# rail-berkeley/serl

Hardware: NVIDIA H100
Metric: drq_critic_grad_steps_per_sec (higher is better)
Workload: dtype f16

## Files before the change

serl_b200/csrc/conv3x3_res.cu:

```cuda
#include "common.cuh"
#include "conv_common.cuh"
#include "serl_b200.h"
#include "wgmma.cuh"

namespace serl {

template <int W, int CI>
struct R3Cfg {
  static constexpr int ROWS = 256 / W;
  static constexpr int BANDS = W / ROWS;
  static constexpr int PARTS = BANDS * (CI / 64);
  static constexpr int CB = CI / 64;
  static constexpr int NBOX = 3 * CB;
  static constexpr int STAGES = CB == 1 ? 3 : 2;
  static constexpr int BOX = W * (ROWS + 2) * 128;
  static constexpr int WTILES = 9 * CB;
  static constexpr int CG = CI / 4;
  static constexpr int NG = 64 / CG;
  static constexpr int WPG = CG / 16;
  static constexpr int PF = 4;
  static constexpr int OFF_A = WTILES * 8192;
  static constexpr int OFF_STG = OFF_A + STAGES * BOX;
  static constexpr int OFF_RED = OFF_STG + 8 * 1024;
  static constexpr int OFF_SLOT = OFF_RED + 2 * 4 * 2 * 4;
  static constexpr int OFF_BAR = OFF_SLOT + 4 * BANDS * NG * 2 * 4;
  static constexpr int SMEM = OFF_BAR + 8 * (2 * STAGES + 5) + 1024;
  static_assert(ROWS * W == 256 && (BOX % 1024) == 0 && SMEM <= 232448, "conv3x3_res_kernel: shared memory layout");
};

struct Res3Args {
  uint16_t* y; const uint16_t* res; const float* gamma; const float* beta;
  const float* res_stats; const float* res_gamma; const float* res_beta;
  int32_t* error; int N, relu; float eps;
};

template <class F, int W, int CI>
__global__ void __launch_bounds__(CONV_THREADS, 1)
conv3x3_res_kernel(const __grid_constant__ CUtensorMap xmap, const __grid_constant__ CUtensorMap wmap, const Res3Args a) {
  pdl_prologue();
  using K = R3Cfg<W, CI>;
  extern __shared__ uint8_t smem_raw[];
  uint8_t* smem = reinterpret_cast<uint8_t*>((reinterpret_cast<uintptr_t>(smem_raw) + 1023) & ~(uintptr_t)1023);
  uint8_t* sW = smem;
  uint8_t* sA = smem + K::OFF_A;
  float* red = reinterpret_cast<float*>(smem + K::OFF_RED);
  float* slot = reinterpret_cast<float*>(smem + K::OFF_SLOT);
  uint64_t* full = reinterpret_cast<uint64_t*>(smem + K::OFF_BAR);
  uint64_t* empty = full + K::STAGES;
  uint64_t* wbar = empty + K::STAGES;
  uint64_t* gnbar = wbar + 1;

  const int warp = threadIdx.x >> 5, lane = threadIdx.x & 31;
  const int part = blockIdx.x % K::PARTS;
  const int band = part % K::BANDS, n0 = (part / K::BANDS) * 64;
  const int row0 = band * K::ROWS;
  const int img0 = blockIdx.x / K::PARTS, img_step = gridDim.x / K::PARTS;

  if (threadIdx.x == 0) {
    for (int s = 0; s < K::STAGES; ++s) { tc_mbar_init(&full[s], 1); tc_mbar_init(&empty[s], 4); }
    tc_mbar_init(wbar, 1);
    for (int q = 0; q < 4; ++q) tc_mbar_init(&gnbar[q], 1);
    asm volatile("fence.mbarrier_init.release.cluster;" ::: "memory");
  }
  __syncthreads();
  if constexpr (K::BANDS > 1) cluster_sync_all();

  if (warp >= 8) {
    asm volatile("setmaxnreg.dec.sync.aligned.u32 40;" ::: "memory");
    if (warp == 8 && lane == 0) {
      asm volatile("prefetch.tensormap [%0];" ::"l"(&xmap) : "memory");
      asm volatile("prefetch.tensormap [%0];" ::"l"(&wmap) : "memory");
      tc_mbar_expect_tx(wbar, (uint32_t)(K::WTILES * 8192));
      for (int t = 0; t < K::WTILES; ++t) tc_tma_2d(sW + t * 8192, &wmap, t * 64, n0, wbar);
      bool ok = true;
      int it = 0;
      for (int n = img0; n < a.N && ok; n += img_step)
        for (int b = 0; b < K::NBOX; ++b, ++it) {
          const int s = it % K::STAGES;
          ok = tc_mbar_wait(&empty[s], ((uint32_t)(it / K::STAGES) & 1u) ^ 1u, a.error);
          if (!ok) break;
          tc_mbar_expect_tx(&full[s], (uint32_t)K::BOX);
          tc_tma_4d(sA + s * K::BOX, &xmap, (b / 3) * 64, b % 3 - 1, row0 - 1, n, &full[s]);
        }
    }
  } else {
    asm volatile("setmaxnreg.inc.sync.aligned.u32 232;" ::: "memory");
    const int g = warp >> 2, wl = warp & 3, tid = threadIdx.x & 127;
    const uint32_t a_base = smem_u32(sA), w_base = smem_u32(sW);
    const float count = (float)(W * W) * (float)K::CG;
    const int grp = wl / K::WPG;
    const int cl = 16 * wl + (lane >> 2);
    uint8_t* stg = smem + K::OFF_STG + warp * 1024;
    const uint32_t mrow = smem_u32(stg) + (uint32_t)(((lane >> 4) * 8 + (lane & 7)) * 32 + ((((lane >> 3) ^ (lane >> 2)) & 1) << 4));
    const int gpx = lane >> 1, gh = lane & 1;
    const uint32_t grow = (uint32_t)(gpx * 32 + ((gh ^ (gpx >> 2)) & 1) * 16);
    bool ok = tc_mbar_wait(wbar, 0u, a.error);
    ok = mma_bar_and(ok);
    float acc[128];
    for (int m = 0;; ++m) {
      const int i = g + 2 * m;
      const int n = img0 + i * img_step;
      if (n >= a.N) break;
      if (i > 0) named_bar_sync(2 + g, 256);
      int it = i * K::NBOX;
      for (int b = 0; b < K::NBOX && ok; ++b, ++it) {
        const int s = it % K::STAGES;
        ok = tc_mbar_wait(&full[s], (uint32_t)(it / K::STAGES) & 1u, a.error);
        if (!ok) break;
        const int cb = b / 3, sx = b % 3;
        const uint32_t bs = a_base + (uint32_t)(s * K::BOX);
        wg_fence();
#pragma unroll
        for (int r = 0; r < 3; ++r) {
          const uint32_t ws = w_base + (uint32_t)(((r * 3 + sx) * K::CB + cb) * 8192);
#pragma unroll
          for (int k = 0; k < 4; ++k)
            wg_mma_h16_n256<F::kBf16>(acc, wg_desc(ws) + 2 * k, wg_desc(bs + (uint32_t)(r * W * 128)) + 2 * k, (uint32_t)(b | r | k));
        }
        wg_commit();
        if (b > 0) {
          wg_wait<1>();
          __syncwarp();
          if (lane == 0) tc_mbar_arrive(&empty[(it - 1) % K::STAGES]);
        }
      }
      if (n + img_step < a.N) named_bar_arrive(3 - g, 256);

      const size_t pix0 = (size_t)n * W * W + (size_t)row0 * W;
      const uint16_t* rsrc = a.res + (pix0 + gpx) * CI + n0 + 16 * wl + 8 * gh;
      uint4 rbuf[K::PF][2];
      if (a.res && ok) {
#pragma unroll
        for (int p = 0; p < K::PF; ++p)
#pragma unroll
          for (int e = 0; e < 2; ++e) rbuf[p][e] = __ldg(reinterpret_cast<const uint4*>(rsrc + (size_t)(32 * p + 16 * e) * CI));
      }
      wg_wait<0>();
      __syncwarp();
      if (ok && lane == 0) tc_mbar_arrive(&empty[(it - 1) % K::STAGES]);

      float S = 0.f, SS = 0.f;
#pragma unroll
      for (int j = 0; j < 32; ++j) {
        const float* d = &acc[4 * j];
        S += (d[0] + d[1]) + (d[2] + d[3]);
        SS += (d[0] * d[0] + d[1] * d[1]) + (d[2] * d[2] + d[3] * d[3]);
      }
      S = warp_sum(S); SS = warp_sum(SS);
      if constexpr (K::WPG > 1) {
        if (lane == 0) *reinterpret_cast<float2*>(red + (g * 4 + wl) * 2) = make_float2(S, SS);
        named_bar_sync(4 + g, 128);
        S = 0.f; SS = 0.f;
#pragma unroll
        for (int k = 0; k < K::WPG; ++k) {
          const float2 v = *reinterpret_cast<const float2*>(red + (g * 4 + grp * K::WPG + k) * 2);
          S += v.x; SS += v.y;
        }
      }
      if constexpr (K::BANDS > 1) {
        const int q = 2 * g + (m & 1);
        if (ok) {
          if (tid == 0) tc_mbar_expect_tx(&gnbar[q], (uint32_t)(K::BANDS * K::NG * 2 * 4));
          if (lane < 2) {
            const float v = lane ? SS : S;
            float* dst = slot + ((q * K::BANDS + band) * K::NG + grp) * 2 + lane;
#pragma unroll
            for (int rk = 0; rk < K::BANDS; ++rk) {
              uint32_t rdst, rbar;
              asm volatile("mapa.shared::cluster.u32 %0, %1, %2;" : "=r"(rdst) : "r"(smem_u32(dst)), "r"(rk));
              asm volatile("mapa.shared::cluster.u32 %0, %1, %2;" : "=r"(rbar) : "r"(smem_u32(&gnbar[q])), "r"(rk));
              asm volatile("st.async.shared::cluster.mbarrier::complete_tx::bytes.b32 [%0], %1, [%2];"
                           ::"r"(rdst), "r"(__float_as_uint(v)), "r"(rbar) : "memory");
            }
          }
          ok = tc_mbar_wait_cluster(&gnbar[q], (uint32_t)(m >> 1) & 1u, a.error);
        }
        S = 0.f; SS = 0.f;
#pragma unroll
        for (int rk = 0; rk < K::BANDS; ++rk) {
          S += slot[((q * K::BANDS + rk) * K::NG + grp) * 2];
          SS += slot[((q * K::BANDS + rk) * K::NG + grp) * 2 + 1];
        }
      }
      if (!ok) continue;

      const float mean = S / count;
      const float var = fmaxf(SS / count - mean * mean, 0.f);
      const float rstd = rsqrtf(var + a.eps);
      float ga[2], gb[2], ra[2] = {1.f, 1.f}, rb[2] = {0.f, 0.f};
#pragma unroll
      for (int h = 0; h < 2; ++h) {
        const int c = n0 + cl + 8 * h;
        ga[h] = rstd * a.gamma[c];
        gb[h] = a.beta[c] - mean * ga[h];
      }
      if (a.res_stats) {
        const int rg = (n0 + cl) / K::CG;
        const float rs = a.res_stats[((size_t)n * 4 + rg) * 2], rss = a.res_stats[((size_t)n * 4 + rg) * 2 + 1];
        const float rmean = rs / count;
        const float rvar = fmaxf(rss / count - rmean * rmean, 0.f);
        const float rrstd = rsqrtf(rvar + a.eps);
#pragma unroll
        for (int h = 0; h < 2; ++h) {
          const int c = n0 + cl + 8 * h;
          ra[h] = rrstd * a.res_gamma[c];
          rb[h] = a.res_beta[c] - rmean * ra[h];
        }
      }

      uint16_t* ydst = a.y + (pix0 + gpx) * CI + n0 + 16 * wl + 8 * gh;
#pragma unroll
      for (int rd = 0; rd < 8; ++rd) {
        uint32_t rv[2][4];
        if (a.res) {
#pragma unroll
          for (int e = 0; e < 2; ++e) *reinterpret_cast<uint4*>(stg + grow + e * 512) = rbuf[rd % K::PF][e];
          __syncwarp();
          ldsm_x4_trans(mrow, rv[0]);
          ldsm_x4_trans(mrow + 512, rv[1]);
          if (rd + K::PF < 8) {
#pragma unroll
            for (int e = 0; e < 2; ++e)
              rbuf[rd % K::PF][e] = __ldg(reinterpret_cast<const uint4*>(rsrc + (size_t)(32 * (rd + K::PF) + 16 * e) * CI));
          }
        }
        uint32_t o[2][4];
#pragma unroll
        for (int x = 0; x < 2; ++x)
#pragma unroll
          for (int jj = 0; jj < 2; ++jj)
#pragma unroll
            for (int h = 0; h < 2; ++h) {
              const float* d = &acc[4 * (4 * rd + 2 * x + jj) + 2 * h];
              float o0 = fmaf(d[0], ga[h], gb[h]), o1 = fmaf(d[1], ga[h], gb[h]);
              if (a.res) {
                const float2 r = F::unpack(rv[x][2 * jj + h]);
                o0 += a.res_stats ? fmaf(r.x, ra[h], rb[h]) : r.x;
                o1 += a.res_stats ? fmaf(r.y, ra[h], rb[h]) : r.y;
              }
              if (a.relu) { o0 = fmaxf(o0, 0.f); o1 = fmaxf(o1, 0.f); }
              o[x][2 * jj + h] = F::pack(o0, o1);
            }
        __syncwarp();
        stsm_x4_trans(mrow, o[0]);
        stsm_x4_trans(mrow + 512, o[1]);
        __syncwarp();
#pragma unroll
        for (int e = 0; e < 2; ++e)
          *reinterpret_cast<uint4*>(ydst + (size_t)(32 * rd + 16 * e) * CI) = *reinterpret_cast<const uint4*>(stg + grow + e * 512);
        __syncwarp();
      }
    }
  }
  if constexpr (K::BANDS > 1) cluster_sync_all();
}

template <class F, int W, int CI>
static int launch_conv3x3_res(const serl_conv3x3_res_desc* d, cudaStream_t st) {
  using K = R3Cfg<W, CI>;
  auto kern = conv3x3_res_kernel<F, W, CI>;
  static int groups = 0;
  if (!groups) {
    if (cudaFuncSetAttribute(kern, cudaFuncAttributeMaxDynamicSharedMemorySize, K::SMEM) != cudaSuccess) return check_launch("cudaFuncSetAttribute(conv3x3_res)");
    int dev = 0, sms = 0, n = 0;
    cudaGetDevice(&dev);
    cudaDeviceGetAttribute(&sms, cudaDevAttrMultiProcessorCount, dev);
    if (K::BANDS > 1) {
      cudaLaunchConfig_t cfg = {};
      cudaLaunchAttribute attr[1];
      attr[0].id = cudaLaunchAttributeClusterDimension;
      attr[0].val.clusterDim.x = K::BANDS; attr[0].val.clusterDim.y = 1; attr[0].val.clusterDim.z = 1;
      cfg.gridDim = dim3(K::BANDS * sms); cfg.blockDim = dim3(CONV_THREADS); cfg.dynamicSmemBytes = K::SMEM;
      cfg.attrs = attr; cfg.numAttrs = 1;
      if (cudaOccupancyMaxActiveClusters(&n, kern, &cfg) != cudaSuccess) return check_launch("cudaOccupancyMaxActiveClusters(conv3x3_res)");
    } else {
      int per_sm = 0;
      if (cudaOccupancyMaxActiveBlocksPerMultiprocessor(&per_sm, kern, CONV_THREADS, K::SMEM) != cudaSuccess) return check_launch("cudaOccupancyMaxActiveBlocksPerMultiprocessor(conv3x3_res)");
      n = per_sm * sms / K::PARTS;
    }
    if (n <= 0) { set_last_error("serl_conv3x3_res_h16: conv3x3_res_kernel (%d B shared memory) cannot be resident", K::SMEM); return SERL_ERR_CUDA; }
    groups = n;
  }
  TcEncodeTiledFn enc = tc_get_encode();
  if (!enc) { set_last_error("serl_conv3x3_res_h16: cuTensorMapEncodeTiled unavailable"); return SERL_ERR_CUDA; }
  const CUtensorMapDataType dt = d->fmt == SERL_FMT_FP16 ? CU_TENSOR_MAP_DATA_TYPE_FLOAT16 : CU_TENSOR_MAP_DATA_TYPE_BFLOAT16;
  CUtensorMap xmap, wmap;
  {
    const cuuint64_t gdim[4] = {(cuuint64_t)CI, (cuuint64_t)W, (cuuint64_t)W, (cuuint64_t)d->N};
    const cuuint64_t gstr[3] = {(cuuint64_t)CI * 2, (cuuint64_t)W * CI * 2, (cuuint64_t)W * W * CI * 2};
    const cuuint32_t box[4] = {64u, (cuuint32_t)W, (cuuint32_t)(K::ROWS + 2), 1u};
    const cuuint32_t estr[4] = {1u, 1u, 1u, 1u};
    CUresult r = enc(&xmap, dt, 4, const_cast<void*>(d->x), gdim, gstr, box, estr, CU_TENSOR_MAP_INTERLEAVE_NONE, CU_TENSOR_MAP_SWIZZLE_128B,
                     CU_TENSOR_MAP_L2_PROMOTION_L2_256B, CU_TENSOR_MAP_FLOAT_OOB_FILL_NONE);
    if (r != CUDA_SUCCESS) { set_last_error("serl_conv3x3_res_h16: cuTensorMapEncodeTiled (input) failed (%d)", (int)r); return SERL_ERR_CUDA; }
  }
  {
    const cuuint64_t gdim[2] = {(cuuint64_t)9 * CI, (cuuint64_t)CI};
    const cuuint64_t gstr[1] = {(cuuint64_t)9 * CI * 2};
    const cuuint32_t box[2] = {64u, 64u};
    const cuuint32_t estr[2] = {1u, 1u};
    CUresult r = enc(&wmap, dt, 2, const_cast<void*>(d->w), gdim, gstr, box, estr, CU_TENSOR_MAP_INTERLEAVE_NONE, CU_TENSOR_MAP_SWIZZLE_128B,
                     CU_TENSOR_MAP_L2_PROMOTION_L2_256B, CU_TENSOR_MAP_FLOAT_OOB_FILL_NONE);
    if (r != CUDA_SUCCESS) { set_last_error("serl_conv3x3_res_h16: cuTensorMapEncodeTiled (weights) failed (%d)", (int)r); return SERL_ERR_CUDA; }
  }
  Res3Args a{};
  a.y = static_cast<uint16_t*>(d->y); a.res = static_cast<const uint16_t*>(d->res); a.gamma = d->gamma; a.beta = d->beta;
  a.res_stats = d->res_stats; a.res_gamma = d->res_gamma; a.res_beta = d->res_beta;
  a.error = d->error; a.N = d->N; a.relu = d->relu; a.eps = d->eps;
  const int rounds = ceil_div(d->N, groups);
  const int used = ceil_div(d->N, rounds);
  launch_k_cluster(kern, dim3(used * K::PARTS), dim3(CONV_THREADS), K::BANDS, (size_t)K::SMEM, st, xmap, wmap, a);
  return check_launch("conv3x3_res_kernel");
}

template <int S, int WO, int CI>
struct PPCfg {
  static constexpr int CO = S * CI;
  static constexpr int HW = WO * WO;
  static constexpr int IMGS = 256 / HW;
  static constexpr int NSL = CO / 64;
  static constexpr int CB = CI / 64;
  static constexpr int NB = S == 2 ? 6 : 3;
  static constexpr int NPH = S == 2 ? 2 : 1;
  static constexpr int BROWS = WO + (S == 2 ? 1 : 2);
  static constexpr int SHIFT = IMGS * WO * 128;
  static constexpr int BOX = BROWS * SHIFT;
  static constexpr int STAGE = BOX + (S == 2 ? 2 : 3) * 8192;
  static constexpr int STAGES = S == 2 ? 4 : 3;
  static constexpr int CG = CO / 4;
  static constexpr int WPG = CG / 16;
  static constexpr int PF = 4;
  static constexpr int OFF_STG = STAGES * STAGE;
  static constexpr int OFF_RED = OFF_STG + 8 * 1024;
  static constexpr int OFF_BAR = OFF_RED + 2 * 2 * 4 * IMGS * 2 * 4;
  static constexpr int SMEM = OFF_BAR + 8 * 2 * STAGES + 1024;
  static_assert(IMGS * HW == 256 && WPG <= 4 && (SHIFT % 1024) == 0 && (STAGE % 1024) == 0 && SMEM <= 232448,
                "conv3x3_pp_kernel: shared memory layout");
  static __host__ __device__ constexpr int nbox(int ph) { return ph ? CB : NB * CB; }
};

struct PPArgs {
  uint16_t* y; uint16_t* r; float* out_f32; const uint16_t* res;
  const float* gamma; const float* beta; const float* gamma_p; const float* beta_p;
  const float* res_stats; const float* res_gamma; const float* res_beta;
  int32_t* error; int N, relu; float eps;
};

template <class F, int S, int WO, int CI>
__global__ void __launch_bounds__(CONV_THREADS, 1)
conv3x3_pp_kernel(const __grid_constant__ CUtensorMap xmap, const __grid_constant__ CUtensorMap wmap,
                  const __grid_constant__ CUtensorMap pmap, const PPArgs a) {
  pdl_prologue();
  using K = PPCfg<S, WO, CI>;
  extern __shared__ uint8_t smem_raw[];
  uint8_t* smem = reinterpret_cast<uint8_t*>((reinterpret_cast<uintptr_t>(smem_raw) + 1023) & ~(uintptr_t)1023);
  float* red = reinterpret_cast<float*>(smem + K::OFF_RED);
  uint64_t* full = reinterpret_cast<uint64_t*>(smem + K::OFF_BAR);
  uint64_t* empty = full + K::STAGES;

  const int warp = threadIdx.x >> 5, lane = threadIdx.x & 31;
  const int n_items = ceil_div(a.N, K::IMGS) * K::NSL;
  auto item_of = [&](int P) {
    const int q = blockIdx.x + ((P & 1) + 2 * ((P >> 1) / K::NPH)) * gridDim.x;
    return P >= 0 && q < n_items ? q : -1;
  };
  auto past_end = [&](int P) { return blockIdx.x + 2 * ((P >> 1) / K::NPH) * gridDim.x >= n_items; };

  if (threadIdx.x == 0) {
    for (int s = 0; s < K::STAGES; ++s) { tc_mbar_init(&full[s], 1); tc_mbar_init(&empty[s], 4); }
    asm volatile("fence.mbarrier_init.release.cluster;" ::: "memory");
  }
  __syncthreads();

  if (warp >= 8) {
    asm volatile("setmaxnreg.dec.sync.aligned.u32 40;" ::: "memory");
    if (warp == 8 && lane == 0) {
      asm volatile("prefetch.tensormap [%0];" ::"l"(&xmap) : "memory");
      asm volatile("prefetch.tensormap [%0];" ::"l"(&wmap) : "memory");
      if (S == 2) asm volatile("prefetch.tensormap [%0];" ::"l"(&pmap) : "memory");
      bool ok = true;
      int it = 0;
      for (int P = 0; ok && !past_end(P); ++P) {
        const int q = item_of(P);
        if (q < 0) continue;
        const int ph = (P >> 1) % K::NPH;
        const int img0 = (q / K::NSL) * K::IMGS, n0 = (q % K::NSL) * 64;
        for (int b = 0; b < K::nbox(ph); ++b, ++it) {
          const int s = it % K::STAGES;
          ok = tc_mbar_wait(&empty[s], ((uint32_t)(it / K::STAGES) & 1u) ^ 1u, a.error);
          if (!ok) break;
          const int cb = ph ? b : b / K::NB, sx = ph ? 0 : b % 3, row0 = S == 2 && !ph ? (b % K::NB) / 3 : 0;
          const int ntap = ph ? 1 : S == 1 ? 3 : row0 == 0 ? 2 : 1;
          uint8_t* st = smem + s * K::STAGE;
          tc_mbar_expect_tx(&full[s], (uint32_t)(K::BOX + ntap * 8192));
          tc_tma_4d(st, &xmap, cb * 64, S == 2 ? sx : sx - 1, img0, S == 2 ? row0 : -1, &full[s]);
          for (int t = 0; t < ntap; ++t) {
            if (ph) tc_tma_2d(st + K::BOX, &pmap, cb * 64, n0, &full[s]);
            else tc_tma_2d(st + K::BOX + t * 8192, &wmap, (((S == 2 ? row0 + 2 * t : t) * 3 + sx) * K::CB + cb) * 64, n0, &full[s]);
          }
        }
      }
    }
  } else {
    asm volatile("setmaxnreg.inc.sync.aligned.u32 232;" ::: "memory");
    const int g = warp >> 2, wl = warp & 3;
    const uint32_t s_base = smem_u32(smem);
    const float count = (float)K::HW * (float)K::CG;
    const int grp = wl / K::WPG;
    const int cl = 16 * wl + (lane >> 2);
    uint8_t* stg = smem + K::OFF_STG + warp * 1024;
    const uint32_t mrow = smem_u32(stg) + (uint32_t)(((lane >> 4) * 8 + (lane & 7)) * 32 + ((((lane >> 3) ^ (lane >> 2)) & 1) << 4));
    const int gpx = lane >> 1, gh = lane & 1;
    const uint32_t grow = (uint32_t)(gpx * 32 + ((gh ^ (gpx >> 2)) & 1) * 16);
    const int pbase = K::IMGS == 1 ? gpx : gpx & 7;
    constexpr int RSTEP = K::IMGS == 1 ? 32 : 8, ESTEP = K::IMGS == 1 ? 16 : 0;
    auto im_of = [&](int e) { return K::IMGS == 1 ? 0 : 2 * e + (gpx >> 3); };
    bool ok = true;
    int it = 0;
    float acc[128];
    for (int P = 0; !past_end(P); ++P) {
      const int q = item_of(P);
      if (q < 0) continue;
      const int k = P >> 1, ph = k % K::NPH;
      if ((P & 1) != g) { it += K::nbox(ph); continue; }
      const int img0 = (q / K::NSL) * K::IMGS, n0 = (q % K::NSL) * 64;
      if (item_of(P - 1) >= 0) named_bar_sync(2 + g, 256);
      if (ph == 0) {
        for (int cb = 0; cb < K::CB && ok; ++cb) {
#pragma unroll
          for (int bb = 0; bb < K::NB; ++bb, ++it) {
            const int s = it % K::STAGES;
            ok = tc_mbar_wait(&full[s], (uint32_t)(it / K::STAGES) & 1u, a.error);
            if (!ok) break;
            const int ntap = S == 1 ? 3 : bb < 3 ? 2 : 1;
            const uint32_t bs = s_base + (uint32_t)(s * K::STAGE), ws = bs + (uint32_t)K::BOX;
            wg_fence();
#pragma unroll
            for (int t = 0; t < ntap; ++t)
#pragma unroll
              for (int kk = 0; kk < 4; ++kk)
                wg_mma_h16_n256<F::kBf16>(acc, wg_desc(ws + (uint32_t)(t * 8192)) + 2 * kk, wg_desc(bs + (uint32_t)(t * K::SHIFT)) + 2 * kk,
                                          (uint32_t)(cb | bb | t | kk));
            wg_commit();
            if (cb > 0 || bb > 0) {
              wg_wait<1>();
              __syncwarp();
              if (lane == 0) tc_mbar_arrive(&empty[(it - 1) % K::STAGES]);
            }
          }
        }
      } else {
        for (int cb = 0; cb < K::CB && ok; ++cb, ++it) {
          const int s = it % K::STAGES;
          ok = tc_mbar_wait(&full[s], (uint32_t)(it / K::STAGES) & 1u, a.error);
          if (!ok) break;
          const uint32_t bs = s_base + (uint32_t)(s * K::STAGE), ws = bs + (uint32_t)K::BOX;
          wg_fence();
#pragma unroll
          for (int kk = 0; kk < 4; ++kk)
            wg_mma_h16_n256<F::kBf16>(acc, wg_desc(ws) + 2 * kk, wg_desc(bs) + 2 * kk, (uint32_t)(cb | kk));
          wg_commit();
          if (cb > 0) {
            wg_wait<1>();
            __syncwarp();
            if (lane == 0) tc_mbar_arrive(&empty[(it - 1) % K::STAGES]);
          }
        }
      }
      if (item_of(P + 1) >= 0) named_bar_arrive(3 - g, 256);

      const uint16_t* rsrc = a.res + ((size_t)img0 * K::HW + pbase) * CI + n0 + 16 * wl + 8 * gh;
      uint4 rbuf[K::PF][2];
      if (S == 1 && a.res && ok) {
#pragma unroll
        for (int p = 0; p < K::PF; ++p)
#pragma unroll
          for (int e = 0; e < 2; ++e)
            rbuf[p][e] = img0 + im_of(e) < a.N ? __ldg(reinterpret_cast<const uint4*>(rsrc + (size_t)(im_of(e) * K::HW + p * RSTEP + e * ESTEP) * CI))
                                               : make_uint4(0u, 0u, 0u, 0u);
      }
      wg_wait<0>();
      __syncwarp();
      if (ok && lane == 0) tc_mbar_arrive(&empty[(it - 1) % K::STAGES]);

      float sm[K::IMGS], ss[K::IMGS];
#pragma unroll
      for (int im = 0; im < K::IMGS; ++im) { sm[im] = 0.f; ss[im] = 0.f; }
#pragma unroll
      for (int j = 0; j < 32; ++j) {
        const float* d = &acc[4 * j];
        sm[j % K::IMGS] += (d[0] + d[1]) + (d[2] + d[3]);
        ss[j % K::IMGS] += (d[0] * d[0] + d[1] * d[1]) + (d[2] * d[2] + d[3] * d[3]);
      }
      float* rw = red + (((k & 1) * 2 + g) * 4) * K::IMGS * 2;
#pragma unroll
      for (int im = 0; im < K::IMGS; ++im) {
        sm[im] = warp_sum(sm[im]); ss[im] = warp_sum(ss[im]);
        if (lane == 0) *reinterpret_cast<float2*>(rw + (wl * K::IMGS + im) * 2) = make_float2(sm[im], ss[im]);
      }
      named_bar_sync(4 + g, 128);
      if (!ok) continue;
      float mean[K::IMGS], rstd[K::IMGS];
#pragma unroll
      for (int im = 0; im < K::IMGS; ++im) {
        float s0 = 0.f, s1 = 0.f;
#pragma unroll
        for (int w = 0; w < K::WPG; ++w) {
          const float2 v = *reinterpret_cast<const float2*>(rw + ((grp * K::WPG + w) * K::IMGS + im) * 2);
          s0 += v.x; s1 += v.y;
        }
        mean[im] = s0 / count;
        rstd[im] = rsqrtf(fmaxf(s1 / count - mean[im] * mean[im], 0.f) + a.eps);
      }

      const float* gam = ph ? a.gamma_p : a.gamma;
      const float* bet = ph ? a.beta_p : a.beta;
      const bool relu = S == 2 ? ph == 0 : a.relu != 0;
      const bool rnorm = S == 1 && a.res_stats;
      float ga[K::IMGS][2], gb[K::IMGS][2], ra[K::IMGS][2], rb[K::IMGS][2];
#pragma unroll
      for (int im = 0; im < K::IMGS; ++im) {
        float rmean = 0.f, rrstd = 1.f;
        if (rnorm && img0 + im < a.N) {
          const float* rs = a.res_stats + ((size_t)(img0 + im) * 4 + n0 / K::CG) * 2;
          rmean = rs[0] / count;
          rrstd = rsqrtf(fmaxf(rs[1] / count - rmean * rmean, 0.f) + a.eps);
        }
#pragma unroll
        for (int h = 0; h < 2; ++h) {
          const int c = n0 + cl + 8 * h;
          ga[im][h] = rstd[im] * gam[c];
          gb[im][h] = bet[c] - mean[im] * ga[im][h];
          ra[im][h] = rnorm ? rrstd * a.res_gamma[c] : 1.f;
          rb[im][h] = rnorm ? a.res_beta[c] - rmean * ra[im][h] : 0.f;
        }
      }

      uint16_t* out = S == 2 && ph ? a.r : a.y;
      const size_t obase = ((size_t)img0 * K::HW + pbase) * K::CO + n0 + 16 * wl + 8 * gh;
#pragma unroll
      for (int rd = 0; rd < 8; ++rd) {
        uint32_t rv[2][4];
        if (S == 1 && a.res) {
#pragma unroll
          for (int e = 0; e < 2; ++e) *reinterpret_cast<uint4*>(stg + grow + e * 512) = rbuf[rd % K::PF][e];
          __syncwarp();
          ldsm_x4_trans(mrow, rv[0]);
          ldsm_x4_trans(mrow + 512, rv[1]);
          if (rd + K::PF < 8) {
#pragma unroll
            for (int e = 0; e < 2; ++e)
              if (img0 + im_of(e) < a.N)
                rbuf[rd % K::PF][e] = __ldg(reinterpret_cast<const uint4*>(rsrc + (size_t)(im_of(e) * K::HW + (rd + K::PF) * RSTEP + e * ESTEP) * CI));
          }
        }
        uint32_t o[2][4];
#pragma unroll
        for (int x = 0; x < 2; ++x)
#pragma unroll
          for (int jj = 0; jj < 2; ++jj) {
            const int j = 4 * rd + 2 * x + jj, im = j % K::IMGS;
#pragma unroll
            for (int h = 0; h < 2; ++h) {
              const float* d = &acc[4 * j + 2 * h];
              float o0 = fmaf(d[0], ga[im][h], gb[im][h]), o1 = fmaf(d[1], ga[im][h], gb[im][h]);
              if (S == 1 && a.res) {
                const float2 r = F::unpack(rv[x][2 * jj + h]);
                o0 += fmaf(r.x, ra[im][h], rb[im][h]);
                o1 += fmaf(r.y, ra[im][h], rb[im][h]);
              }
              if (relu) { o0 = fmaxf(o0, 0.f); o1 = fmaxf(o1, 0.f); }
              if (S == 1 && a.out_f32 && img0 + im < a.N) {
                float* of = a.out_f32 + ((size_t)(img0 + im) * K::HW + 8 * (j / K::IMGS) + 2 * (lane & 3)) * CI + n0 + cl + 8 * h;
                of[0] = o0;
                of[CI] = o1;
              }
              o[x][2 * jj + h] = F::pack(o0, o1);
            }
          }
        __syncwarp();
        if (S == 2 || !a.out_f32) {
          stsm_x4_trans(mrow, o[0]);
          stsm_x4_trans(mrow + 512, o[1]);
          __syncwarp();
#pragma unroll
          for (int e = 0; e < 2; ++e)
            if (img0 + im_of(e) < a.N)
              *reinterpret_cast<uint4*>(out + obase + (size_t)(im_of(e) * K::HW + rd * RSTEP + e * ESTEP) * K::CO) =
                  *reinterpret_cast<const uint4*>(stg + grow + e * 512);
          __syncwarp();
        }
      }
    }
  }
}

template <class F, int S, int WO, int CI>
static int launch_conv3x3_pp(const char* name, const void* x, const void* w, const void* w_proj, int fmt, const PPArgs& a, cudaStream_t st) {
  using K = PPCfg<S, WO, CI>;
  auto kern = conv3x3_pp_kernel<F, S, WO, CI>;
  static int slots = 0;
  if (!slots) {
    if (cudaFuncSetAttribute(kern, cudaFuncAttributeMaxDynamicSharedMemorySize, K::SMEM) != cudaSuccess) return check_launch("cudaFuncSetAttribute(conv3x3_pp)");
    int dev = 0, sms = 0, per_sm = 0;
    cudaGetDevice(&dev);
    cudaDeviceGetAttribute(&sms, cudaDevAttrMultiProcessorCount, dev);
    if (cudaOccupancyMaxActiveBlocksPerMultiprocessor(&per_sm, kern, CONV_THREADS, K::SMEM) != cudaSuccess) return check_launch("cudaOccupancyMaxActiveBlocksPerMultiprocessor(conv3x3_pp)");
    if (per_sm <= 0) { set_last_error("%s: conv3x3_pp_kernel (%d B shared memory) cannot be resident", name, K::SMEM); return SERL_ERR_CUDA; }
    slots = per_sm * sms;
  }
  TcEncodeTiledFn enc = tc_get_encode();
  if (!enc) { set_last_error("%s: cuTensorMapEncodeTiled unavailable", name); return SERL_ERR_CUDA; }
  const CUtensorMapDataType dt = fmt == SERL_FMT_FP16 ? CU_TENSOR_MAP_DATA_TYPE_FLOAT16 : CU_TENSOR_MAP_DATA_TYPE_BFLOAT16;
  CUtensorMap xmap, wmap, pmap;
  {
    constexpr int WI = S * WO;
    const cuuint64_t gdim[4] = {(cuuint64_t)CI, (cuuint64_t)WI, (cuuint64_t)a.N, (cuuint64_t)WI};
    const cuuint64_t gstr[3] = {(cuuint64_t)CI * 2, (cuuint64_t)WI * WI * CI * 2, (cuuint64_t)WI * CI * 2};
    const cuuint32_t box[4] = {64u, (cuuint32_t)(S * WO), (cuuint32_t)K::IMGS, (cuuint32_t)(S * K::BROWS)};
    const cuuint32_t estr[4] = {1u, (cuuint32_t)S, 1u, (cuuint32_t)S};
    CUresult r = enc(&xmap, dt, 4, const_cast<void*>(x), gdim, gstr, box, estr, CU_TENSOR_MAP_INTERLEAVE_NONE, CU_TENSOR_MAP_SWIZZLE_128B,
                     CU_TENSOR_MAP_L2_PROMOTION_L2_256B, CU_TENSOR_MAP_FLOAT_OOB_FILL_NONE);
    if (r != CUDA_SUCCESS) { set_last_error("%s: cuTensorMapEncodeTiled (input) failed (%d)", name, (int)r); return SERL_ERR_CUDA; }
  }
  for (int pj = 0; pj < S; ++pj) {
    const cuuint64_t kdim = (cuuint64_t)(pj ? 1 : 9) * CI;
    const cuuint64_t gdim[2] = {kdim, (cuuint64_t)K::CO};
    const cuuint64_t gstr[1] = {kdim * 2};
    const cuuint32_t box[2] = {64u, 64u};
    const cuuint32_t estr[2] = {1u, 1u};
    CUresult r = enc(pj ? &pmap : &wmap, dt, 2, const_cast<void*>(pj ? w_proj : w), gdim, gstr, box, estr, CU_TENSOR_MAP_INTERLEAVE_NONE,
                     CU_TENSOR_MAP_SWIZZLE_128B, CU_TENSOR_MAP_L2_PROMOTION_L2_256B, CU_TENSOR_MAP_FLOAT_OOB_FILL_NONE);
    if (r != CUDA_SUCCESS) { set_last_error("%s: cuTensorMapEncodeTiled (weights) failed (%d)", name, (int)r); return SERL_ERR_CUDA; }
  }
  if (S == 1) pmap = wmap;
  const int items = ceil_div(a.N, K::IMGS) * K::NSL;
  const int rounds = ceil_div(items, slots);
  launch_k(kern, dim3(ceil_div(items, rounds)), dim3(CONV_THREADS), (size_t)K::SMEM, st, xmap, wmap, pmap, a);
  return check_launch("conv3x3_pp_kernel");
}

template <class F, int WO, int CI>
static int launch_conv3x3s2_pp(const serl_conv3x3s2_res_desc* d, cudaStream_t st) {
  PPArgs a{};
  a.y = static_cast<uint16_t*>(d->y); a.r = static_cast<uint16_t*>(d->r);
  a.gamma = d->gamma; a.beta = d->beta; a.gamma_p = d->gamma_proj; a.beta_p = d->beta_proj;
  a.error = d->error; a.N = d->N; a.relu = 1; a.eps = d->eps;
  return launch_conv3x3_pp<F, 2, WO, CI>("serl_conv3x3s2_res_h16", d->x, d->w, d->w_proj, d->fmt, a, st);
}

template <class F>
static int launch_conv3x3_res8_pp(const serl_conv3x3_res_desc* d, cudaStream_t st) {
  PPArgs a{};
  a.out_f32 = d->out_f32; a.y = d->out_f32 ? nullptr : static_cast<uint16_t*>(d->y);
  a.res = static_cast<const uint16_t*>(d->res); a.gamma = d->gamma; a.beta = d->beta;
  a.res_stats = d->res_stats; a.res_gamma = d->res_gamma; a.res_beta = d->res_beta;
  a.error = d->error; a.N = d->N; a.relu = d->relu; a.eps = d->eps;
  return launch_conv3x3_pp<F, 1, 8, 256>("serl_conv3x3_res_h16", d->x, d->w, nullptr, d->fmt, a, st);
}

template <int WO, int CI>
struct S2Cfg {
  static constexpr int CO = 2 * CI;
  static constexpr int BN = 128;
  static constexpr int M = 128;
  static constexpr int HW = WO * WO;
  static constexpr int IMGS = M / HW;
  static constexpr int NSL = CO / BN;
  static constexpr int CB = CI / 64;
  static constexpr int NB = 9;
  static constexpr int NBOX = NB * CB;
  static constexpr int BOX = IMGS * HW * 128;
  static constexpr int TILE = BN * 128;
  static constexpr int STAGE = BOX + 2 * TILE;
  static constexpr int STAGES = 4;
  static constexpr int CG = CO / 4;
  static constexpr int CGS = 64;
  static constexpr int GPS = 64 / CGS;
  static constexpr int NGC = BN / CG;
  static constexpr int OFF_STG = STAGES * STAGE;
  static constexpr int OFF_PAR = OFF_STG + 8 * 1024;
  static constexpr int OFF_RED = OFF_PAR + BN * 16;
  static constexpr int OFF_ST = OFF_RED + 8 * 2 * GPS * 16;
  static constexpr int OFF_BAR = OFF_ST + IMGS * NGC * 16;
  static constexpr int SMEM = OFF_BAR + 8 * 2 * STAGES + 1024;
  static_assert(WO == 4 && BN % CG == 0, "conv3x3s2_res_kernel: the WO 4 head, an item holds whole GroupNorm groups");
  static_assert(M % HW == 0 && (BOX % 1024) == 0 && (STAGE % 1024) == 0 && SMEM <= 232448, "conv3x3s2_res_kernel: shared memory layout");
  __device__ static constexpr int m_off(int wg, int) { return wg * 64; }
  __device__ static constexpr int n_off(int h) { return h * 64; }
};

struct S2Args {
  uint16_t* y; uint16_t* r; const float* gamma; const float* beta; const float* gamma_p; const float* beta_p;
  int32_t* error; int N; float eps;
};

template <class F, int WO, int CI>
__global__ void __launch_bounds__(CONV_THREADS, 1)
conv3x3s2_res_kernel(const __grid_constant__ CUtensorMap xmap, const __grid_constant__ CUtensorMap wmap,
                     const __grid_constant__ CUtensorMap pmap, const S2Args a) {
  pdl_prologue();
  using K = S2Cfg<WO, CI>;
  extern __shared__ uint8_t smem_raw[];
  uint8_t* smem = reinterpret_cast<uint8_t*>((reinterpret_cast<uintptr_t>(smem_raw) + 1023) & ~(uintptr_t)1023);
  float* par = reinterpret_cast<float*>(smem + K::OFF_PAR);
  float* red = reinterpret_cast<float*>(smem + K::OFF_RED);
  float* gst = reinterpret_cast<float*>(smem + K::OFF_ST);
  uint64_t* full = reinterpret_cast<uint64_t*>(smem + K::OFF_BAR);
  uint64_t* empty = full + K::STAGES;

  const int warp = threadIdx.x >> 5, lane = threadIdx.x & 31;
  const int n_items = ceil_div(a.N, K::IMGS) * K::NSL;

  if (threadIdx.x == 0) {
    for (int s = 0; s < K::STAGES; ++s) { tc_mbar_init(&full[s], 1); tc_mbar_init(&empty[s], 8); }
    asm volatile("fence.mbarrier_init.release.cluster;" ::: "memory");
  }
  __syncthreads();

  if (warp >= 8) {
    asm volatile("setmaxnreg.dec.sync.aligned.u32 40;" ::: "memory");
    if (warp == 8 && lane == 0) {
      asm volatile("prefetch.tensormap [%0];" ::"l"(&xmap) : "memory");
      asm volatile("prefetch.tensormap [%0];" ::"l"(&wmap) : "memory");
      asm volatile("prefetch.tensormap [%0];" ::"l"(&pmap) : "memory");
      bool ok = true;
      int it = 0;
      for (int item = blockIdx.x; item < n_items && ok; item += gridDim.x) {
        const int img = (item / K::NSL) * K::IMGS, n0 = (item % K::NSL) * K::BN;
        for (int b = 0; b < K::NBOX; ++b, ++it) {
          const int s = it % K::STAGES;
          ok = tc_mbar_wait(&empty[s], ((uint32_t)(it / K::STAGES) & 1u) ^ 1u, a.error);
          if (!ok) break;
          const int cb = b / K::NB, row = (b % K::NB) / 3, sx = b % 3;
          const bool proj = row == 0 && sx == 0;
          uint8_t* st = smem + s * K::STAGE;
          tc_mbar_expect_tx(&full[s], (uint32_t)(K::BOX + (1 + (int)proj) * K::TILE));
          tc_tma_4d(st, &xmap, cb * 64, sx, row, img, &full[s]);
          tc_tma_2d(st + K::BOX, &wmap, ((row * 3 + sx) * K::CB + cb) * 64, n0, &full[s]);
          if (proj) tc_tma_2d(st + K::BOX + K::TILE, &pmap, cb * 64, n0, &full[s]);
        }
      }
    }
  } else {
    asm volatile("setmaxnreg.inc.sync.aligned.u32 232;" ::: "memory");
    const int tid = threadIdx.x, wg = tid >> 7, wl = warp & 3;
    const uint32_t s_base = smem_u32(smem);
    uint32_t a_off[2], b_off[2];
#pragma unroll
    for (int h = 0; h < 2; ++h) {
      const int m = K::m_off(wg, h);
      a_off[h] = (uint32_t)(m * 128);
      b_off[h] = (uint32_t)(K::n_off(h) * 128);
    }
    const float count = (float)K::HW * (float)K::CG;
    bool ok = true;
    int it = 0;
    float acc[2][32], pacc[2][32];
    for (int item = blockIdx.x; item < n_items && ok; item += gridDim.x) {
      const int img0 = (item / K::NSL) * K::IMGS, n0 = (item % K::NSL) * K::BN;
      for (int cb = 0; cb < K::CB && ok; ++cb) {
#pragma unroll
        for (int bb = 0; bb < K::NB; ++bb, ++it) {
          const int s = it % K::STAGES;
          ok = tc_mbar_wait(&full[s], (uint32_t)(it / K::STAGES) & 1u, a.error);
          if (!ok) break;
          const uint32_t as = s_base + (uint32_t)(s * K::STAGE), ws = as + (uint32_t)K::BOX;
          wg_fence();
#pragma unroll
          for (int k = 0; k < 4; ++k)
#pragma unroll
            for (int h = 0; h < 2; ++h)
              wg_mma_h16<F::kBf16>(acc[h], wg_desc(as + a_off[h]) + 2 * k, wg_desc(ws + b_off[h]) + 2 * k, (uint32_t)(cb | bb | k));
          if (bb == 0) {
#pragma unroll
            for (int k = 0; k < 4; ++k)
#pragma unroll
              for (int h = 0; h < 2; ++h)
                wg_mma_h16<F::kBf16>(pacc[h], wg_desc(as + a_off[h]) + 2 * k, wg_desc(ws + (uint32_t)K::TILE + b_off[h]) + 2 * k,
                                     (uint32_t)(cb | k));
          }
          wg_commit();
          if (cb > 0 || bb > 0) {
            wg_wait<1>();
            __syncwarp();
            if (lane == 0) tc_mbar_arrive(&empty[(it - 1) % K::STAGES]);
          }
        }
      }
      wg_wait<0>();
      ok = mma_bar_and(ok);
      if (!ok) break;
      __syncwarp();
      if (lane == 0) tc_mbar_arrive(&empty[(it - 1) % K::STAGES]);

#pragma unroll
      for (int h = 0; h < 2; ++h)
#pragma unroll
        for (int g = 0; g < K::GPS; ++g) {
          float v[4] = {0.f, 0.f, 0.f, 0.f};
#pragma unroll
          for (int j = g * K::CGS / 8; j < (g + 1) * K::CGS / 8; ++j) {
            const float* d = &acc[h][4 * j];
            const float* p = &pacc[h][4 * j];
            v[0] += (d[0] + d[1]) + (d[2] + d[3]);
            v[1] += (d[0] * d[0] + d[1] * d[1]) + (d[2] * d[2] + d[3] * d[3]);
            v[2] += (p[0] + p[1]) + (p[2] + p[3]);
            v[3] += (p[0] * p[0] + p[1] * p[1]) + (p[2] * p[2] + p[3] * p[3]);
          }
#pragma unroll
          for (int q = 0; q < 4; ++q) {
            v[q] = warp_sum(v[q]);
            if (lane == 0) red[((warp * 2 + h) * K::GPS + g) * 4 + q] = v[q];
          }
        }
      asm volatile("bar.sync 1, 256;" ::: "memory");
      if (tid < K::BN)
        *reinterpret_cast<float4*>(par + tid * 4) = make_float4(a.gamma[n0 + tid], a.beta[n0 + tid], a.gamma_p[n0 + tid], a.beta_p[n0 + tid]);
      if (tid < K::IMGS * K::NGC) {
        const int im = tid / K::NGC, gc = tid % K::NGC;
        float S[4] = {0.f, 0.f, 0.f, 0.f};
        for (int w = 0; w < 8; ++w)
          for (int h = 0; h < 2; ++h)
            for (int g = 0; g < K::GPS; ++g) {
              if ((K::m_off(w >> 2, h) + 16 * (w & 3)) / K::HW != im || (K::n_off(h) + g * K::CGS) / K::CG != gc) continue;
              for (int q = 0; q < 4; ++q) S[q] += red[((w * 2 + h) * K::GPS + g) * 4 + q];
            }
        const float mean = S[0] / count, pmean = S[2] / count;
        const float var = fmaxf(S[1] / count - mean * mean, 0.f), pvar = fmaxf(S[3] / count - pmean * pmean, 0.f);
        *reinterpret_cast<float4*>(gst + tid * 4) = make_float4(mean, rsqrtf(var + a.eps), pmean, rsqrtf(pvar + a.eps));
      }
      asm volatile("bar.sync 1, 256;" ::: "memory");

      uint8_t* stg = smem + K::OFF_STG + warp * 1024;
#pragma unroll
      for (int h = 0; h < 2; ++h)
#pragma unroll
        for (int hf = 0; hf < 2; ++hf) {
          const int m8 = K::m_off(wg, h) + wl * 16 + hf * 8;
          const int im = m8 / K::HW;
          if (img0 + im >= a.N) continue;
          const int rr = lane >> 2;
          const size_t pix0 = (size_t)img0 * K::HW + m8;
#pragma unroll 1
          for (int o = 0; o < 2; ++o) {
#pragma unroll
            for (int j = 0; j < 8; ++j) {
              const int c = K::n_off(h) + 8 * j + 2 * (lane & 3);
              const float4 sv = *reinterpret_cast<const float4*>(gst + (im * K::NGC + c / K::CG) * 4);
              const float4 p0 = *reinterpret_cast<const float4*>(par + c * 4), p1 = *reinterpret_cast<const float4*>(par + c * 4 + 4);
              float o0, o1;
              if (o == 0) {
                const float g0 = sv.y * p0.x, g1 = sv.y * p1.x;
                o0 = fmaxf(fmaf(acc[h][4 * j + 2 * hf], g0, p0.y - sv.x * g0), 0.f);
                o1 = fmaxf(fmaf(acc[h][4 * j + 2 * hf + 1], g1, p1.y - sv.x * g1), 0.f);
              } else {
                const float g0 = sv.w * p0.z, g1 = sv.w * p1.z;
                o0 = fmaf(pacc[h][4 * j + 2 * hf], g0, p0.w - sv.z * g0);
                o1 = fmaf(pacc[h][4 * j + 2 * hf + 1], g1, p1.w - sv.z * g1);
              }
              *reinterpret_cast<uint32_t*>(stg + rr * 128 + ((j ^ rr) << 4) + (lane & 3) * 4) = F::pack(o0, o1);
            }
            __syncwarp();
            uint16_t* out = o == 0 ? a.y : a.r;
#pragma unroll
            for (int e = lane; e < 64; e += 32) {
              const int q = e >> 3, ch = e & 7;
              const uint4 v = *reinterpret_cast<const uint4*>(stg + q * 128 + ((ch ^ q) << 4));
              *reinterpret_cast<uint4*>(out + (pix0 + q) * K::CO + n0 + K::n_off(h) + ch * 8) = v;
            }
            __syncwarp();
          }
        }
    }
  }
}

template <class F, int WO, int CI>
static int launch_conv3x3s2_res(const serl_conv3x3s2_res_desc* d, cudaStream_t st) {
  using K = S2Cfg<WO, CI>;
  auto kern = conv3x3s2_res_kernel<F, WO, CI>;
  static int slots = 0;
  if (!slots) {
    if (cudaFuncSetAttribute(kern, cudaFuncAttributeMaxDynamicSharedMemorySize, K::SMEM) != cudaSuccess) return check_launch("cudaFuncSetAttribute(conv3x3s2_res)");
    int dev = 0, sms = 0, per_sm = 0;
    cudaGetDevice(&dev);
    cudaDeviceGetAttribute(&sms, cudaDevAttrMultiProcessorCount, dev);
    if (cudaOccupancyMaxActiveBlocksPerMultiprocessor(&per_sm, kern, CONV_THREADS, K::SMEM) != cudaSuccess) return check_launch("cudaOccupancyMaxActiveBlocksPerMultiprocessor(conv3x3s2_res)");
    if (per_sm <= 0) { set_last_error("serl_conv3x3s2_res_h16: conv3x3s2_res_kernel (%d B shared memory) cannot be resident", K::SMEM); return SERL_ERR_CUDA; }
    slots = per_sm * sms;
  }
  TcEncodeTiledFn enc = tc_get_encode();
  if (!enc) { set_last_error("serl_conv3x3s2_res_h16: cuTensorMapEncodeTiled unavailable"); return SERL_ERR_CUDA; }
  const CUtensorMapDataType dt = d->fmt == SERL_FMT_FP16 ? CU_TENSOR_MAP_DATA_TYPE_FLOAT16 : CU_TENSOR_MAP_DATA_TYPE_BFLOAT16;
  CUtensorMap xmap, wmap, pmap;
  {
    const cuuint64_t gdim[4] = {(cuuint64_t)CI, (cuuint64_t)(2 * WO), (cuuint64_t)(2 * WO), (cuuint64_t)d->N};
    const cuuint64_t gstr[3] = {(cuuint64_t)CI * 2, (cuuint64_t)2 * WO * CI * 2, (cuuint64_t)4 * WO * WO * CI * 2};
    const cuuint32_t box[4] = {64u, (cuuint32_t)(2 * WO), (cuuint32_t)(2 * WO), (cuuint32_t)K::IMGS};
    const cuuint32_t estr[4] = {1u, 2u, 2u, 1u};
    CUresult r = enc(&xmap, dt, 4, const_cast<void*>(d->x), gdim, gstr, box, estr, CU_TENSOR_MAP_INTERLEAVE_NONE, CU_TENSOR_MAP_SWIZZLE_128B,
                     CU_TENSOR_MAP_L2_PROMOTION_L2_256B, CU_TENSOR_MAP_FLOAT_OOB_FILL_NONE);
    if (r != CUDA_SUCCESS) { set_last_error("serl_conv3x3s2_res_h16: cuTensorMapEncodeTiled (input) failed (%d)", (int)r); return SERL_ERR_CUDA; }
  }
  for (int pj = 0; pj < 2; ++pj) {
    const cuuint64_t kdim = (cuuint64_t)(pj ? 1 : 9) * CI;
    const cuuint64_t gdim[2] = {kdim, (cuuint64_t)K::CO};
    const cuuint64_t gstr[1] = {kdim * 2};
    const cuuint32_t box[2] = {64u, (cuuint32_t)K::BN};
    const cuuint32_t estr[2] = {1u, 1u};
    CUresult r = enc(pj ? &pmap : &wmap, dt, 2, const_cast<void*>(pj ? d->w_proj : d->w), gdim, gstr, box, estr, CU_TENSOR_MAP_INTERLEAVE_NONE,
                     CU_TENSOR_MAP_SWIZZLE_128B, CU_TENSOR_MAP_L2_PROMOTION_L2_256B, CU_TENSOR_MAP_FLOAT_OOB_FILL_NONE);
    if (r != CUDA_SUCCESS) { set_last_error("serl_conv3x3s2_res_h16: cuTensorMapEncodeTiled (weights) failed (%d)", (int)r); return SERL_ERR_CUDA; }
  }
  S2Args a{};
  a.y = static_cast<uint16_t*>(d->y); a.r = static_cast<uint16_t*>(d->r);
  a.gamma = d->gamma; a.beta = d->beta; a.gamma_p = d->gamma_proj; a.beta_p = d->beta_proj;
  a.error = d->error; a.N = d->N; a.eps = d->eps;
  const int items = ceil_div(d->N, K::IMGS) * K::NSL;
  const int rounds = ceil_div(items, slots);
  launch_k(kern, dim3(ceil_div(items, rounds)), dim3(CONV_THREADS), (size_t)K::SMEM, st, xmap, wmap, pmap, a);
  return check_launch("conv3x3s2_res_kernel");
}

template <int W, int CI>
struct DeepCfg {
  static constexpr int BN = 128;
  static constexpr int HW = W * W;
  static constexpr int IMGS = 256 / HW;
  static constexpr int NSL = CI / BN;
  static constexpr int CB = CI / 64;
  static constexpr int NB = 9;
  static constexpr int NBOX = NB * CB;
  static constexpr int BOX = IMGS * HW * 128;
  static constexpr int TILE = BN * 128;
  static constexpr int STAGE = BOX + TILE;
  static constexpr int STAGES = 4;
  static constexpr int RES = 128 * 128 * 2;
  static constexpr int RPS = STAGE / RES;
  static constexpr int NRES = 2 / RPS;
  static constexpr int CG = CI / 4;
  static constexpr int NGC = BN / CG;
  static constexpr int OFF_STG = STAGES * STAGE;
  static constexpr int OFF_PAR = OFF_STG + 8 * 2048;
  static constexpr int OFF_RED = OFF_PAR + BN * 16;
  static constexpr int OFF_ST = OFF_RED + 8 * 2 * 2 * 8;
  static constexpr int OFF_BAR = OFF_ST + IMGS * NGC * 16;
  static constexpr int SMEM = OFF_BAR + 8 * 2 * STAGES + 1024;
  static_assert(CG >= 64 && BN % CG == 0, "conv3x3_deep_kernel: an n64 sub-tile lies in one group, an item holds whole groups");
  static_assert(RPS >= 1 && NRES < STAGES, "conv3x3_deep_kernel: the residual fits the ring");
  static_assert(HW >= 16 && (BOX % 1024) == 0 && (STAGE % 1024) == 0 && SMEM <= 232448, "conv3x3_deep_kernel: shared memory layout");
  __device__ static constexpr int m_off(int wg, int h) { return wg * 128 + h * 64; }
};

struct DeepArgs {
  uint16_t* y; float* out_f32; const uint16_t* res; const float* gamma; const float* beta;
  const float* res_stats; const float* res_gamma; const float* res_beta;
  int32_t* error; int N, relu; float eps;
};

template <class F, int W, int CI>
__global__ void __launch_bounds__(CONV_THREADS, 1)
conv3x3_deep_kernel(const __grid_constant__ CUtensorMap xmap, const __grid_constant__ CUtensorMap wmap,
                    const __grid_constant__ CUtensorMap rmap, const DeepArgs a) {
  pdl_prologue();
  using K = DeepCfg<W, CI>;
  extern __shared__ uint8_t smem_raw[];
  uint8_t* smem = reinterpret_cast<uint8_t*>((reinterpret_cast<uintptr_t>(smem_raw) + 1023) & ~(uintptr_t)1023);
  float* par = reinterpret_cast<float*>(smem + K::OFF_PAR);
  float* red = reinterpret_cast<float*>(smem + K::OFF_RED);
  float* gst = reinterpret_cast<float*>(smem + K::OFF_ST);
  uint64_t* full = reinterpret_cast<uint64_t*>(smem + K::OFF_BAR);
  uint64_t* empty = full + K::STAGES;

  const int warp = threadIdx.x >> 5, lane = threadIdx.x & 31;
  const int n_items = ceil_div(a.N, K::IMGS) * K::NSL;

  if (threadIdx.x == 0) {
    for (int s = 0; s < K::STAGES; ++s) { tc_mbar_init(&full[s], 1); tc_mbar_init(&empty[s], 8); }
    asm volatile("fence.mbarrier_init.release.cluster;" ::: "memory");
  }
  __syncthreads();

  if (warp >= 8) {
    asm volatile("setmaxnreg.dec.sync.aligned.u32 40;" ::: "memory");
    if (warp == 8 && lane == 0) {
      asm volatile("prefetch.tensormap [%0];" ::"l"(&xmap) : "memory");
      asm volatile("prefetch.tensormap [%0];" ::"l"(&wmap) : "memory");
      if (a.res) asm volatile("prefetch.tensormap [%0];" ::"l"(&rmap) : "memory");
      bool ok = true;
      int it = 0;
      for (int item = blockIdx.x; item < n_items && ok; item += gridDim.x) {
        const int img = (item / K::NSL) * K::IMGS, n0 = (item % K::NSL) * K::BN;
        for (int b = 0; b < K::NBOX + (a.res ? K::NRES : 0); ++b, ++it) {
          const int s = it % K::STAGES;
          ok = tc_mbar_wait(&empty[s], ((uint32_t)(it / K::STAGES) & 1u) ^ 1u, a.error);
          if (!ok) break;
          uint8_t* st = smem + s * K::STAGE;
          if (b >= K::NBOX) {
            tc_mbar_expect_tx(&full[s], (uint32_t)(K::RPS * K::RES));
            for (int q = 0; q < K::RPS; ++q)
              for (int c = 0; c < 2; ++c)
                tc_tma_2d(st + q * K::RES + c * (K::RES / 2), &rmap, n0 + c * 64, img * K::HW + ((b - K::NBOX) * K::RPS + q) * 128, &full[s]);
            continue;
          }
          const int cb = b / K::NB, row = (b % K::NB) / 3, sx = b % 3;
          tc_mbar_expect_tx(&full[s], (uint32_t)K::STAGE);
          tc_tma_4d(st, &xmap, cb * 64, sx - 1, row - 1, img, &full[s]);
          tc_tma_2d(st + K::BOX, &wmap, ((row * 3 + sx) * K::CB + cb) * 64, n0, &full[s]);
        }
      }
    }
  } else {
    asm volatile("setmaxnreg.inc.sync.aligned.u32 232;" ::: "memory");
    const int tid = threadIdx.x, wg = tid >> 7, wl = warp & 3;
    const uint32_t s_base = smem_u32(smem);
    uint32_t a_off[2];
#pragma unroll
    for (int h = 0; h < 2; ++h) a_off[h] = (uint32_t)(K::m_off(wg, h) * 128);
    const float count = (float)K::HW * (float)K::CG;
    bool ok = true;
    int it = 0;
    float acc[2][2][32];
    for (int item = blockIdx.x; item < n_items && ok; item += gridDim.x) {
      const int img0 = (item / K::NSL) * K::IMGS, n0 = (item % K::NSL) * K::BN;
      for (int cb = 0; cb < K::CB && ok; ++cb) {
#pragma unroll
        for (int bb = 0; bb < K::NB; ++bb, ++it) {
          const int s = it % K::STAGES;
          ok = tc_mbar_wait(&full[s], (uint32_t)(it / K::STAGES) & 1u, a.error);
          if (!ok) break;
          const uint32_t as = s_base + (uint32_t)(s * K::STAGE), ws = as + (uint32_t)K::BOX;
          wg_fence();
#pragma unroll
          for (int k = 0; k < 4; ++k)
#pragma unroll
            for (int h = 0; h < 2; ++h)
#pragma unroll
              for (int c = 0; c < 2; ++c)
                wg_mma_h16<F::kBf16>(acc[h][c], wg_desc(as + a_off[h]) + 2 * k, wg_desc(ws + (uint32_t)(c * 64 * 128)) + 2 * k,
                                     (uint32_t)(cb | bb | k));
          wg_commit();
          if (cb > 0 || bb > 0) {
            wg_wait<1>();
            __syncwarp();
            if (lane == 0) tc_mbar_arrive(&empty[(it - 1) % K::STAGES]);
          }
        }
      }
      wg_wait<0>();
      ok = mma_bar_and(ok);
      if (!ok) break;
      __syncwarp();
      if (lane == 0) tc_mbar_arrive(&empty[(it - 1) % K::STAGES]);

#pragma unroll
      for (int h = 0; h < 2; ++h)
#pragma unroll
        for (int c = 0; c < 2; ++c) {
          float v0 = 0.f, v1 = 0.f;
#pragma unroll
          for (int j = 0; j < 8; ++j) {
            const float* d = &acc[h][c][4 * j];
            v0 += (d[0] + d[1]) + (d[2] + d[3]);
            v1 += (d[0] * d[0] + d[1] * d[1]) + (d[2] * d[2] + d[3] * d[3]);
          }
          v0 = warp_sum(v0); v1 = warp_sum(v1);
          if (lane == 0) *reinterpret_cast<float2*>(red + ((warp * 2 + h) * 2 + c) * 2) = make_float2(v0, v1);
        }
      asm volatile("bar.sync 1, 256;" ::: "memory");
      if (tid < K::BN) {
        const int ch = n0 + tid;
        *reinterpret_cast<float4*>(par + tid * 4) = a.res_stats ? make_float4(a.gamma[ch], a.beta[ch], a.res_gamma[ch], a.res_beta[ch])
                                                                : make_float4(a.gamma[ch], a.beta[ch], 1.f, 0.f);
      }
      if (tid < K::IMGS * K::NGC) {
        const int im = tid / K::NGC, gc = tid % K::NGC;
        float S = 0.f, SS = 0.f;
        for (int w = 0; w < 8; ++w)
          for (int h = 0; h < 2; ++h)
            for (int c = 0; c < 2; ++c) {
              if ((K::m_off(w >> 2, h) + 16 * (w & 3)) / K::HW != im || c * 64 / K::CG != gc) continue;
              S += red[((w * 2 + h) * 2 + c) * 2];
              SS += red[((w * 2 + h) * 2 + c) * 2 + 1];
            }
        const float mean = S / count;
        const float var = fmaxf(SS / count - mean * mean, 0.f);
        float rmean = 0.f, rrstd = 1.f;
        if (a.res_stats && img0 + im < a.N) {
          const float* rs = a.res_stats + ((size_t)(img0 + im) * 4 + (n0 / K::CG + gc)) * 2;
          rmean = rs[0] / count;
          rrstd = rsqrtf(fmaxf(rs[1] / count - rmean * rmean, 0.f) + a.eps);
        }
        *reinterpret_cast<float4*>(gst + tid * 4) = make_float4(mean, rsqrtf(var + a.eps), rmean, rrstd);
      }
      const int rpos = it + wg / K::RPS;
      const uint8_t* rsm = smem + (rpos % K::STAGES) * K::STAGE + (wg % K::RPS) * K::RES;
      if (a.res) ok = tc_mbar_wait(&full[rpos % K::STAGES], (uint32_t)(rpos / K::STAGES) & 1u, a.error);
      ok = mma_bar_and(ok);
      if (!ok) break;

      uint8_t* stg = smem + K::OFF_STG + warp * 2048;
      const int rr = lane >> 2;
#pragma unroll
      for (int h = 0; h < 2; ++h)
#pragma unroll
        for (int hf = 0; hf < 2; ++hf) {
          const int m8 = K::m_off(wg, h) + wl * 16 + hf * 8;
          const int im = m8 / K::HW;
          if (img0 + im >= a.N) continue;
          const size_t pix0 = (size_t)img0 * K::HW + m8;
#pragma unroll
          for (int c = 0; c < 2; ++c) {
            const float4 sv = *reinterpret_cast<const float4*>(gst + (im * K::NGC + c * 64 / K::CG) * 4);
#pragma unroll
            for (int j = 0; j < 8; ++j) {
              const int cl = c * 64 + 8 * j + 2 * (lane & 3);
              const float4 p0 = *reinterpret_cast<const float4*>(par + cl * 4), p1 = *reinterpret_cast<const float4*>(par + cl * 4 + 4);
              const float g0 = sv.y * p0.x, g1 = sv.y * p1.x;
              float o0 = fmaf(acc[h][c][4 * j + 2 * hf], g0, p0.y - sv.x * g0);
              float o1 = fmaf(acc[h][c][4 * j + 2 * hf + 1], g1, p1.y - sv.x * g1);
              if (a.res) {
                const float2 rv = F::unpack(*reinterpret_cast<const uint32_t*>(
                    rsm + c * (K::RES / 2) + (m8 - wg * 128 + rr) * 128 + ((j ^ rr) << 4) + (lane & 3) * 4));
                if (a.res_stats) {
                  const float r0 = sv.w * p0.z, r1 = sv.w * p1.z;
                  o0 += fmaf(rv.x, r0, p0.w - sv.z * r0);
                  o1 += fmaf(rv.y, r1, p1.w - sv.z * r1);
                } else {
                  o0 += rv.x; o1 += rv.y;
                }
              }
              if (a.relu) { o0 = fmaxf(o0, 0.f); o1 = fmaxf(o1, 0.f); }
              if (a.out_f32)
                *reinterpret_cast<float2*>(stg + rr * 256 + ((j ^ rr) << 5) + (lane & 3) * 8) = make_float2(o0, o1);
              else
                *reinterpret_cast<uint32_t*>(stg + rr * 128 + ((j ^ rr) << 4) + (lane & 3) * 4) = F::pack(o0, o1);
            }
            __syncwarp();
            if (a.out_f32) {
#pragma unroll
              for (int e = lane; e < 128; e += 32) {
                const int q = e >> 4, ch = e & 15;
                const uint4 v = *reinterpret_cast<const uint4*>(stg + q * 256 + (((ch >> 1) ^ q) << 5) + (ch & 1) * 16);
                *reinterpret_cast<uint4*>(a.out_f32 + (pix0 + q) * CI + n0 + c * 64 + ch * 4) = v;
              }
            } else {
#pragma unroll
              for (int e = lane; e < 64; e += 32) {
                const int q = e >> 3, ch = e & 7;
                const uint4 v = *reinterpret_cast<const uint4*>(stg + q * 128 + ((ch ^ q) << 4));
                *reinterpret_cast<uint4*>(a.y + (pix0 + q) * CI + n0 + c * 64 + ch * 8) = v;
              }
            }
            __syncwarp();
          }
        }
      if (a.res) {
        __syncwarp();
        if (lane == 0)
          for (int p = 0; p < K::NRES; ++p) tc_mbar_arrive(&empty[(it + p) % K::STAGES]);
        it += K::NRES;
      }
    }
  }
}

template <class F, int W, int CI>
static int launch_conv3x3_deep(const serl_conv3x3_res_desc* d, cudaStream_t st) {
  using K = DeepCfg<W, CI>;
  auto kern = conv3x3_deep_kernel<F, W, CI>;
  static int slots = 0;
  if (!slots) {
    if (cudaFuncSetAttribute(kern, cudaFuncAttributeMaxDynamicSharedMemorySize, K::SMEM) != cudaSuccess) return check_launch("cudaFuncSetAttribute(conv3x3_deep)");
    int dev = 0, sms = 0, per_sm = 0;
    cudaGetDevice(&dev);
    cudaDeviceGetAttribute(&sms, cudaDevAttrMultiProcessorCount, dev);
    if (cudaOccupancyMaxActiveBlocksPerMultiprocessor(&per_sm, kern, CONV_THREADS, K::SMEM) != cudaSuccess) return check_launch("cudaOccupancyMaxActiveBlocksPerMultiprocessor(conv3x3_deep)");
    if (per_sm <= 0) { set_last_error("serl_conv3x3_res_h16: conv3x3_deep_kernel (%d B shared memory) cannot be resident", K::SMEM); return SERL_ERR_CUDA; }
    slots = per_sm * sms;
  }
  TcEncodeTiledFn enc = tc_get_encode();
  if (!enc) { set_last_error("serl_conv3x3_res_h16: cuTensorMapEncodeTiled unavailable"); return SERL_ERR_CUDA; }
  const CUtensorMapDataType dt = d->fmt == SERL_FMT_FP16 ? CU_TENSOR_MAP_DATA_TYPE_FLOAT16 : CU_TENSOR_MAP_DATA_TYPE_BFLOAT16;
  CUtensorMap xmap, wmap, rmap;
  {
    const cuuint64_t gdim[4] = {(cuuint64_t)CI, (cuuint64_t)W, (cuuint64_t)W, (cuuint64_t)d->N};
    const cuuint64_t gstr[3] = {(cuuint64_t)CI * 2, (cuuint64_t)W * CI * 2, (cuuint64_t)W * W * CI * 2};
    const cuuint32_t box[4] = {64u, (cuuint32_t)W, (cuuint32_t)W, (cuuint32_t)K::IMGS};
    const cuuint32_t estr[4] = {1u, 1u, 1u, 1u};
    CUresult r = enc(&xmap, dt, 4, const_cast<void*>(d->x), gdim, gstr, box, estr, CU_TENSOR_MAP_INTERLEAVE_NONE, CU_TENSOR_MAP_SWIZZLE_128B,
                     CU_TENSOR_MAP_L2_PROMOTION_L2_256B, CU_TENSOR_MAP_FLOAT_OOB_FILL_NONE);
    if (r != CUDA_SUCCESS) { set_last_error("serl_conv3x3_res_h16: cuTensorMapEncodeTiled (input) failed (%d)", (int)r); return SERL_ERR_CUDA; }
  }
  {
    const cuuint64_t gdim[2] = {(cuuint64_t)9 * CI, (cuuint64_t)CI};
    const cuuint64_t gstr[1] = {(cuuint64_t)9 * CI * 2};
    const cuuint32_t box[2] = {64u, (cuuint32_t)K::BN};
    const cuuint32_t estr[2] = {1u, 1u};
    CUresult r = enc(&wmap, dt, 2, const_cast<void*>(d->w), gdim, gstr, box, estr, CU_TENSOR_MAP_INTERLEAVE_NONE, CU_TENSOR_MAP_SWIZZLE_128B,
                     CU_TENSOR_MAP_L2_PROMOTION_L2_256B, CU_TENSOR_MAP_FLOAT_OOB_FILL_NONE);
    if (r != CUDA_SUCCESS) { set_last_error("serl_conv3x3_res_h16: cuTensorMapEncodeTiled (weights) failed (%d)", (int)r); return SERL_ERR_CUDA; }
  }
  rmap = wmap;
  if (d->res) {
    const cuuint64_t gdim[2] = {(cuuint64_t)CI, (cuuint64_t)d->N * W * W};
    const cuuint64_t gstr[1] = {(cuuint64_t)CI * 2};
    const cuuint32_t box[2] = {64u, 128u};
    const cuuint32_t estr[2] = {1u, 1u};
    CUresult r = enc(&rmap, dt, 2, const_cast<void*>(d->res), gdim, gstr, box, estr, CU_TENSOR_MAP_INTERLEAVE_NONE, CU_TENSOR_MAP_SWIZZLE_128B,
                     CU_TENSOR_MAP_L2_PROMOTION_L2_256B, CU_TENSOR_MAP_FLOAT_OOB_FILL_NONE);
    if (r != CUDA_SUCCESS) { set_last_error("serl_conv3x3_res_h16: cuTensorMapEncodeTiled (residual) failed (%d)", (int)r); return SERL_ERR_CUDA; }
  }
  DeepArgs a{};
  a.out_f32 = d->out_f32; a.y = d->out_f32 ? nullptr : static_cast<uint16_t*>(d->y);
  a.res = static_cast<const uint16_t*>(d->res); a.gamma = d->gamma; a.beta = d->beta;
  a.res_stats = d->res_stats; a.res_gamma = d->res_gamma; a.res_beta = d->res_beta;
  a.error = d->error; a.N = d->N; a.relu = d->relu; a.eps = d->eps;
  const int items = ceil_div(d->N, K::IMGS) * K::NSL;
  const int rounds = ceil_div(items, slots);
  launch_k(kern, dim3(ceil_div(items, rounds)), dim3(CONV_THREADS), (size_t)K::SMEM, st, xmap, wmap, rmap, a);
  return check_launch("conv3x3_deep_kernel");
}

}

using namespace serl;

extern "C" int serl_conv3x3s2_res_h16(const serl_conv3x3s2_res_desc* d, void* stream) {
  if (!d || !d->x || !d->w || !d->w_proj || !d->y || !d->r || !d->gamma || !d->beta || !d->gamma_proj || !d->beta_proj || !d->error || d->N < 1) {
    set_last_error("serl_conv3x3s2_res_h16: invalid descriptor"); return SERL_ERR_INVALID;
  }
  if (d->Co != 2 * d->Ci) { set_last_error("serl_conv3x3s2_res_h16: Co == 2 Ci only (ResNet-10 stage heads)"); return SERL_ERR_UNSUPPORTED; }
  if (!((d->Wo == 16 && d->Co == 128) || (d->Wo == 8 && d->Co == 256) || (d->Wo == 4 && d->Co == 512))) {
    set_last_error("serl_conv3x3s2_res_h16: unsupported shape (Wo=%d, Ci=%d, Co=%d)", d->Wo, d->Ci, d->Co); return SERL_ERR_UNSUPPORTED;
  }
  const bool h = d->fmt == SERL_FMT_FP16;
  const cudaStream_t st = static_cast<cudaStream_t>(stream);
  if (d->Wo == 16) return h ? launch_conv3x3s2_pp<Fp16, 16, 64>(d, st) : launch_conv3x3s2_pp<Bf16, 16, 64>(d, st);
  if (d->Wo == 8) return h ? launch_conv3x3s2_pp<Fp16, 8, 128>(d, st) : launch_conv3x3s2_pp<Bf16, 8, 128>(d, st);
  return h ? launch_conv3x3s2_res<Fp16, 4, 256>(d, st) : launch_conv3x3s2_res<Bf16, 4, 256>(d, st);
}

extern "C" int serl_conv3x3_res_h16(const serl_conv3x3_res_desc* d, void* stream) {
  if (!d || !d->x || !d->w || !d->gamma || !d->beta || !d->error || (!d->y && !d->out_f32) || d->N < 1) {
    set_last_error("serl_conv3x3_res_h16: invalid descriptor"); return SERL_ERR_INVALID;
  }
  if ((d->res_stats != nullptr) != (d->res_gamma != nullptr) || (d->res_stats != nullptr) != (d->res_beta != nullptr) || (d->res_stats && !d->res)) {
    set_last_error("serl_conv3x3_res_h16: res_stats / res_gamma / res_beta go together (and need res)"); return SERL_ERR_INVALID;
  }
  if (d->H != d->W || d->Co != d->Ci) { set_last_error("serl_conv3x3_res_h16: square maps with Ci == Co only"); return SERL_ERR_UNSUPPORTED; }
  if (!((d->W == 32 && d->Ci == 64) || (d->W == 16 && d->Ci == 128) || (d->W == 8 && d->Ci == 256) || (d->W == 4 && d->Ci == 512))) {
    set_last_error("serl_conv3x3_res_h16: unsupported shape (H=W=%d, Ci=%d, Co=%d): ResNet-10 block shapes at 128x128 input only", d->W, d->Ci, d->Co);
    return SERL_ERR_UNSUPPORTED;
  }
  if (d->out_f32 && d->W >= 16) {
    set_last_error("serl_conv3x3_res_h16: out_f32 at 8x8 and 4x4 only"); return SERL_ERR_UNSUPPORTED;
  }
  if (d->W == 32) {
    return d->fmt == SERL_FMT_FP16 ? launch_conv3x3_res<Fp16, 32, 64>(d, static_cast<cudaStream_t>(stream))
                                   : launch_conv3x3_res<Bf16, 32, 64>(d, static_cast<cudaStream_t>(stream));
  }
  if (d->W == 16) {
    return d->fmt == SERL_FMT_FP16 ? launch_conv3x3_res<Fp16, 16, 128>(d, static_cast<cudaStream_t>(stream))
                                   : launch_conv3x3_res<Bf16, 16, 128>(d, static_cast<cudaStream_t>(stream));
  }
  if (d->W == 8) {
    return d->fmt == SERL_FMT_FP16 ? launch_conv3x3_res8_pp<Fp16>(d, static_cast<cudaStream_t>(stream))
                                   : launch_conv3x3_res8_pp<Bf16>(d, static_cast<cudaStream_t>(stream));
  }
  return d->fmt == SERL_FMT_FP16 ? launch_conv3x3_deep<Fp16, 4, 512>(d, static_cast<cudaStream_t>(stream))
                                 : launch_conv3x3_deep<Bf16, 4, 512>(d, static_cast<cudaStream_t>(stream));
}
```

serl_b200/csrc/conv_common.cuh:

```cuda
#pragma once
#include <cuda.h>
#include <cuda_bf16.h>
#include <cuda_fp16.h>
#include <stdint.h>

#include "common.cuh"

namespace serl {

__device__ inline uint32_t smem_u32(const void* p) { return (uint32_t)__cvta_generic_to_shared(p); }

__device__ inline void tc_mbar_init(uint64_t* bar, int count) {
  asm volatile("mbarrier.init.shared::cta.b64 [%0], %1;" ::"r"(smem_u32(bar)), "r"(count));
}
__device__ inline void tc_mbar_arrive(uint64_t* bar) {
  asm volatile("mbarrier.arrive.shared::cta.b64 _, [%0];" ::"r"(smem_u32(bar)) : "memory");
}
__device__ inline bool tc_mbar_wait(uint64_t* bar, uint32_t parity, int32_t* error) {
  const uint32_t addr = smem_u32(bar);
  const long long t0 = clock64();
#pragma unroll 1
  for (;;) {
    uint32_t done;
    asm volatile("{\n .reg .pred p;\n mbarrier.try_wait.parity.shared::cta.b64 p, [%1], %2;\n selp.u32 %0, 1, 0, p;\n}"
                 : "=r"(done) : "r"(addr), "r"(parity) : "memory");
    if (done) return true;
    if (clock64() - t0 > 4000000000ll) break;
  }
  atomicOr(error, 2);
  return false;
}
__device__ inline bool tc_mbar_wait_cluster(uint64_t* bar, uint32_t parity, int32_t* error) {
  const uint32_t addr = smem_u32(bar);
  const long long t0 = clock64();
#pragma unroll 1
  for (;;) {
    uint32_t done;
    asm volatile("{\n .reg .pred p;\n mbarrier.try_wait.parity.acquire.cluster.shared::cta.b64 p, [%1], %2;\n selp.u32 %0, 1, 0, p;\n}"
                 : "=r"(done) : "r"(addr), "r"(parity) : "memory");
    if (done) return true;
    if (clock64() - t0 > 4000000000ll) break;
  }
  atomicOr(error, 2);
  return false;
}

struct Bf16 {
  static constexpr bool kBf16 = true;
  __device__ static inline uint32_t pack(float lo, float hi) { __nv_bfloat162 v = __floats2bfloat162_rn(lo, hi); return *reinterpret_cast<uint32_t*>(&v); }
  __device__ static inline float2 unpack(uint32_t u) { return __bfloat1622float2(*reinterpret_cast<__nv_bfloat162*>(&u)); }
  __device__ static inline uint32_t max2(uint32_t a, uint32_t b) {
    __nv_bfloat162 r = __hmax2(*reinterpret_cast<__nv_bfloat162*>(&a), *reinterpret_cast<__nv_bfloat162*>(&b)); return *reinterpret_cast<uint32_t*>(&r);
  }
};
struct Fp16 {
  static constexpr bool kBf16 = false;
  __device__ static inline uint32_t pack(float lo, float hi) {
    __half2 v = __floats2half2_rn(fminf(fmaxf(lo, -65504.f), 65504.f), fminf(fmaxf(hi, -65504.f), 65504.f));
    return *reinterpret_cast<uint32_t*>(&v);
  }
  __device__ static inline float2 unpack(uint32_t u) { return __half22float2(*reinterpret_cast<__half2*>(&u)); }
  __device__ static inline uint32_t max2(uint32_t a, uint32_t b) {
    __half2 r = __hmax2(*reinterpret_cast<__half2*>(&a), *reinterpret_cast<__half2*>(&b)); return *reinterpret_cast<uint32_t*>(&r);
  }
};
template <class F>
__device__ inline uint32_t affine_relu_x2(uint32_t u, float a0, float b0, float a1, float b1) {
  float2 f = F::unpack(u);
  return F::pack(fmaxf(fmaf(f.x, a0, b0), 0.f), fmaxf(fmaf(f.y, a1, b1), 0.f));
}

__device__ inline void tc_mbar_expect_tx(uint64_t* bar, uint32_t bytes) {
  asm volatile("mbarrier.arrive.expect_tx.shared::cta.b64 _, [%0], %1;" ::"r"(smem_u32(bar)), "r"(bytes) : "memory");
}
__device__ inline void tc_tma_2d(void* smem_dst, const CUtensorMap* map, int c0, int c1, uint64_t* bar) {
  asm volatile("cp.async.bulk.tensor.2d.shared::cluster.global.tile.mbarrier::complete_tx::bytes [%0], [%1, {%3, %4}], [%2];"
               ::"r"(smem_u32(smem_dst)), "l"(map), "r"(smem_u32(bar)), "r"(c0), "r"(c1) : "memory");
}
__device__ inline void tc_tma_4d(void* smem_dst, const CUtensorMap* map, int c0, int c1, int c2, int c3, uint64_t* bar) {
  asm volatile("cp.async.bulk.tensor.4d.shared::cluster.global.tile.mbarrier::complete_tx::bytes [%0], [%1, {%3, %4, %5, %6}], [%2];"
               ::"r"(smem_u32(smem_dst)), "l"(map), "r"(smem_u32(bar)), "r"(c0), "r"(c1), "r"(c2), "r"(c3) : "memory");
}

constexpr int CONV_THREADS = 384;

__device__ inline bool mma_bar_and(bool v) {
  uint32_t r;
  asm volatile("{\n .reg .pred p, q;\n setp.ne.u32 p, %1, 0;\n barrier.red.and.pred q, 1, 256, p;\n selp.u32 %0, 1, 0, q;\n}"
               : "=r"(r) : "r"((uint32_t)v) : "memory");
  return r != 0;
}
__device__ inline void cluster_sync_all() {
  asm volatile("barrier.cluster.arrive.release;\n barrier.cluster.wait.acquire;" ::: "memory");
}
__device__ inline void named_bar_sync(int id, int threads) { asm volatile("bar.sync %0, %1;" ::"r"(id), "r"(threads) : "memory"); }
__device__ inline void named_bar_arrive(int id, int threads) { asm volatile("bar.arrive %0, %1;" ::"r"(id), "r"(threads) : "memory"); }
__device__ inline void ldsm_x4_trans(uint32_t addr, uint32_t (&r)[4]) {
  asm volatile("ldmatrix.sync.aligned.m8n8.x4.trans.shared.b16 {%0, %1, %2, %3}, [%4];"
               : "=r"(r[0]), "=r"(r[1]), "=r"(r[2]), "=r"(r[3]) : "r"(addr) : "memory");
}
__device__ inline void stsm_x4_trans(uint32_t addr, const uint32_t (&r)[4]) {
  asm volatile("stmatrix.sync.aligned.m8n8.x4.trans.shared.b16 [%0], {%1, %2, %3, %4};"
               ::"r"(addr), "r"(r[0]), "r"(r[1]), "r"(r[2]), "r"(r[3]) : "memory");
}

struct GnSrc {
  const float* a; const float* b;
  const float* stats; const float* gamma; const float* beta;
  float count, eps; int Cg;
};
__device__ inline void gn_load8(const GnSrc& g, int n, int C, int c0, float (&a)[8], float (&b)[8]) {
  if (g.stats) {
    const int grp = c0 / g.Cg;
    const float s = g.stats[((size_t)n * 4 + grp) * 2], ss = g.stats[((size_t)n * 4 + grp) * 2 + 1];
    const float mean = s / g.count;
    const float var = fmaxf(ss / g.count - mean * mean, 0.f);
    const float rstd = rsqrtf(var + g.eps);
    const float4 g0 = *reinterpret_cast<const float4*>(g.gamma + c0), g1 = *reinterpret_cast<const float4*>(g.gamma + c0 + 4);
    const float4 e0 = *reinterpret_cast<const float4*>(g.beta + c0), e1 = *reinterpret_cast<const float4*>(g.beta + c0 + 4);
    const float gm[8] = {g0.x, g0.y, g0.z, g0.w, g1.x, g1.y, g1.z, g1.w}, bt[8] = {e0.x, e0.y, e0.z, e0.w, e1.x, e1.y, e1.z, e1.w};
#pragma unroll
    for (int j = 0; j < 8; ++j) { a[j] = rstd * gm[j]; b[j] = bt[j] - mean * a[j]; }
  } else {
    const size_t co = (size_t)n * C + c0;
    const float4 a0 = *reinterpret_cast<const float4*>(g.a + co), a1 = *reinterpret_cast<const float4*>(g.a + co + 4);
    const float4 b0 = *reinterpret_cast<const float4*>(g.b + co), b1 = *reinterpret_cast<const float4*>(g.b + co + 4);
    a[0] = a0.x; a[1] = a0.y; a[2] = a0.z; a[3] = a0.w; a[4] = a1.x; a[5] = a1.y; a[6] = a1.z; a[7] = a1.w;
    b[0] = b0.x; b[1] = b0.y; b[2] = b0.z; b[3] = b0.w; b[4] = b1.x; b[5] = b1.y; b[6] = b1.z; b[7] = b1.w;
  }
}

typedef CUresult (*TcEncodeTiledFn)(CUtensorMap*, CUtensorMapDataType, cuuint32_t, void*, const cuuint64_t*, const cuuint64_t*,
                                    const cuuint32_t*, const cuuint32_t*, CUtensorMapInterleave, CUtensorMapSwizzle,
                                    CUtensorMapL2promotion, CUtensorMapFloatOOBfill);
inline TcEncodeTiledFn tc_get_encode() {
  static TcEncodeTiledFn fn = nullptr;
  if (!fn) {
    void* p = nullptr;
    cudaDriverEntryPointQueryResult qres;
    if (cudaGetDriverEntryPoint("cuTensorMapEncodeTiled", &p, cudaEnableDefault, &qres) == cudaSuccess && qres == cudaDriverEntryPointSuccess)
      fn = reinterpret_cast<TcEncodeTiledFn>(p);
  }
  return fn;
}

}
```

Before: 541.9.

## Extend pp conv kernel to 4x4 maps with 2-CTA cluster multicast

Generalizes the pipelined conv3x3 kernel so it also covers the 4x4 spatial (and 8x8 deep residual) layers. For 4x4 outputs it uses 2-CTA clusters that split output channel slices, alternately multicasting the shared input box via TMA to both CTAs, and exchanging group-norm partial sums across CTAs with st.async. It replaces the dedicated deep/res8/s2_res kernels. The added cross-CTA barrier traffic and remote arrivals add synchronization cost and complexity in exchange for less duplicated input loading and a unified kernel.

```diff
diff --git a/serl_b200/csrc/conv3x3_res.cu b/serl_b200/csrc/conv3x3_res.cu
--- a/serl_b200/csrc/conv3x3_res.cu
+++ b/serl_b200/csrc/conv3x3_res.cu
@@ -326,16 +326,23 @@
   static constexpr int SHIFT = IMGS * WO * 128;
   static constexpr int BOX = BROWS * SHIFT;
   static constexpr int STAGE = BOX + (S == 2 ? 2 : 3) * 8192;
-  static constexpr int STAGES = S == 2 ? 4 : 3;
+  static constexpr int STAGES = S == 2 && WO > 4 ? 4 : 3;
+  static constexpr int CL = WO == 4 ? 2 : 1;
+  static constexpr int NU = NSL / CL;
   static constexpr int CG = CO / 4;
   static constexpr int WPG = CG / 16;
-  static constexpr int PF = 4;
+  static constexpr bool XG = WPG > 4;
+  static constexpr int GW = XG ? 4 : WPG;
+  static constexpr int TI = WO >= 8 ? IMGS : IMGS / 2;
+  static constexpr int PF = WO >= 8 ? 4 : 1;
   static constexpr int OFF_STG = STAGES * STAGE;
+  static constexpr int RSL = XG ? 1 : 2;
   static constexpr int OFF_RED = OFF_STG + 8 * 1024;
-  static constexpr int OFF_BAR = OFF_RED + 2 * 2 * 4 * IMGS * 2 * 4;
-  static constexpr int SMEM = OFF_BAR + 8 * 2 * STAGES + 1024;
-  static_assert(IMGS * HW == 256 && WPG <= 4 && (SHIFT % 1024) == 0 && (STAGE % 1024) == 0 && SMEM <= 232448,
-                "conv3x3_pp_kernel: shared memory layout");
+  static constexpr int OFF_XCH = OFF_RED + RSL * 2 * 4 * IMGS * 2 * 4;
+  static constexpr int OFF_BAR = OFF_XCH + (XG ? 2 * 2 * IMGS * 2 * 4 : 0);
+  static constexpr int SMEM = OFF_BAR + 8 * (2 * STAGES + (XG ? 4 : 0)) + 1024;
+  static_assert(IMGS * HW == 256 && NSL % CL == 0 && (WPG <= 4 || (WPG == 8 && CL == 2)) && (SHIFT % 1024) == 0 &&
+                (STAGE % 1024) == 0 && SMEM <= 232448, "conv3x3_pp_kernel: shared memory layout");
   static __host__ __device__ constexpr int nbox(int ph) { return ph ? CB : NB * CB; }
 };
 
@@ -345,6 +352,14 @@
   const float* res_stats; const float* res_gamma; const float* res_beta;
   int32_t* error; int N, relu; float eps;
 };
+
+__device__ inline float warp_sum_skip2(float v) {
+  v += __shfl_xor_sync(0xffffffffu, v, 16);
+  v += __shfl_xor_sync(0xffffffffu, v, 8);
+  v += __shfl_xor_sync(0xffffffffu, v, 4);
+  v += __shfl_xor_sync(0xffffffffu, v, 1);
+  return v;
+}
 
 template <class F, int S, int WO, int CI>
 __global__ void __launch_bounds__(CONV_THREADS, 1)
@@ -355,22 +370,27 @@
   extern __shared__ uint8_t smem_raw[];
   uint8_t* smem = reinterpret_cast<uint8_t*>((reinterpret_cast<uintptr_t>(smem_raw) + 1023) & ~(uintptr_t)1023);
   float* red = reinterpret_cast<float*>(smem + K::OFF_RED);
+  float* xch = reinterpret_cast<float*>(smem + K::OFF_XCH);
   uint64_t* full = reinterpret_cast<uint64_t*>(smem + K::OFF_BAR);
   uint64_t* empty = full + K::STAGES;
+  uint64_t* xbar = empty + K::STAGES;
 
   const int warp = threadIdx.x >> 5, lane = threadIdx.x & 31;
-  const int n_items = ceil_div(a.N, K::IMGS) * K::NSL;
+  const int rank = blockIdx.x % K::CL;
   auto item_of = [&](int P) {
-    const int q = blockIdx.x + ((P & 1) + 2 * ((P >> 1) / K::NPH)) * gridDim.x;
-    return P >= 0 && q < n_items ? q : -1;
+    const int q = blockIdx.x / K::CL + ((P & 1) + 2 * ((P >> 1) / K::NPH)) * (gridDim.x / K::CL);
+    return P >= 0 && q < ceil_div(a.N, K::IMGS) * K::NU ? q : -1;
   };
-  auto past_end = [&](int P) { return blockIdx.x + 2 * ((P >> 1) / K::NPH) * gridDim.x >= n_items; };
+  auto past_end = [&](int P) { return blockIdx.x / K::CL + 2 * ((P >> 1) / K::NPH) * (gridDim.x / K::CL) >= ceil_div(a.N, K::IMGS) * K::NU; };
+  auto slice0 = [&](int q) { return (K::CL * (q % K::NU) + rank) * 64; };
 
   if (threadIdx.x == 0) {
-    for (int s = 0; s < K::STAGES; ++s) { tc_mbar_init(&full[s], 1); tc_mbar_init(&empty[s], 4); }
+    for (int s = 0; s < K::STAGES; ++s) { tc_mbar_init(&full[s], 1); tc_mbar_init(&empty[s], 4 * K::CL); }
+    if (K::XG) for (int q = 0; q < 4; ++q) tc_mbar_init(&xbar[q], 1);
     asm volatile("fence.mbarrier_init.release.cluster;" ::: "memory");
   }
   __syncthreads();
+  if constexpr (K::CL > 1) cluster_sync_all();
 
   if (warp >= 8) {
     asm volatile("setmaxnreg.dec.sync.aligned.u32 40;" ::: "memory");
@@ -384,16 +404,18 @@
         const int q = item_of(P);
         if (q < 0) continue;
         const int ph = (P >> 1) % K::NPH;
-        const int img0 = (q / K::NSL) * K::IMGS, n0 = (q % K::NSL) * 64;
+        const int img0 = (q / K::NU) * K::IMGS, n0 = slice0(q);
         for (int b = 0; b < K::nbox(ph); ++b, ++it) {
           const int s = it % K::STAGES;
-          ok = tc_mbar_wait(&empty[s], ((uint32_t)(it / K::STAGES) & 1u) ^ 1u, a.error);
+          const uint32_t par = ((uint32_t)(it / K::STAGES) & 1u) ^ 1u;
+          ok = tc_mbar_wait(&empty[s], par, a.error);
           if (!ok) break;
           const int cb = ph ? b : b / K::NB, sx = ph ? 0 : b % 3, row0 = S == 2 && !ph ? (b % K::NB) / 3 : 0;
           const int ntap = ph ? 1 : S == 1 ? 3 : row0 == 0 ? 2 : 1;
           uint8_t* st = smem + s * K::STAGE;
           tc_mbar_expect_tx(&full[s], (uint32_t)(K::BOX + ntap * 8192));
-          tc_tma_4d(st, &xmap, cb * 64, S == 2 ? sx : sx - 1, img0, S == 2 ? row0 : -1, &full[s]);
+          if constexpr (K::CL == 1) tc_tma_4d(st, &xmap, cb * 64, S == 2 ? sx : sx - 1, img0, S == 2 ? row0 : -1, &full[s]);
+          else if ((it & 1) == rank) tc_tma_4d_mc(st, &xmap, cb * 64, S == 2 ? sx : sx - 1, img0, S == 2 ? row0 : -1, &full[s], (uint16_t)3u);
           for (int t = 0; t < ntap; ++t) {
             if (ph) tc_tma_2d(st + K::BOX, &pmap, cb * 64, n0, &full[s]);
             else tc_tma_2d(st + K::BOX + t * 8192, &wmap, (((S == 2 ? row0 + 2 * t : t) * 3 + sx) * K::CB + cb) * 64, n0, &full[s]);
@@ -403,18 +425,27 @@
     }
   } else {
     asm volatile("setmaxnreg.inc.sync.aligned.u32 232;" ::: "memory");
-    const int g = warp >> 2, wl = warp & 3;
+    const int g = warp >> 2, wl = warp & 3, tid = threadIdx.x & 127;
     const uint32_t s_base = smem_u32(smem);
     const float count = (float)K::HW * (float)K::CG;
     const int grp = wl / K::WPG;
     const int cl = 16 * wl + (lane >> 2);
+    const int lb = (lane >> 1) & 1;
+    auto img_of = [&](int t) { return WO >= 8 ? t : 2 * t + lb; };
+    auto release = [&](int pos) {
+      tc_mbar_arrive(&empty[pos % K::STAGES]);
+      if constexpr (K::CL > 1) tc_mbar_arrive_remote(&empty[pos % K::STAGES], (uint32_t)(rank ^ 1));
+    };
     uint8_t* stg = smem + K::OFF_STG + warp * 1024;
     const uint32_t mrow = smem_u32(stg) + (uint32_t)(((lane >> 4) * 8 + (lane & 7)) * 32 + ((((lane >> 3) ^ (lane >> 2)) & 1) << 4));
     const int gpx = lane >> 1, gh = lane & 1;
     const uint32_t grow = (uint32_t)(gpx * 32 + ((gh ^ (gpx >> 2)) & 1) * 16);
-    const int pbase = K::IMGS == 1 ? gpx : gpx & 7;
-    constexpr int RSTEP = K::IMGS == 1 ? 32 : 8, ESTEP = K::IMGS == 1 ? 16 : 0;
-    auto im_of = [&](int e) { return K::IMGS == 1 ? 0 : 2 * e + (gpx >> 3); };
+    const int lim = (gpx / WO) % K::IMGS, lpx = lim * K::HW + gpx % WO;
+    auto rimg = [&](int rd, int e) { return (32 * rd / WO + 16 * e / WO) % K::IMGS + lim; };
+    auto rpix = [&](int rd, int e) {
+      return ((32 * rd / WO + 16 * e / WO) % K::IMGS) * K::HW + ((32 * rd + 16 * e) / (K::IMGS * WO)) * WO + lpx;
+    };
+    const int fpx = 2 * (lane & 3) % WO;
     bool ok = true;
     int it = 0;
     float acc[128];
@@ -423,7 +454,7 @@
       if (q < 0) continue;
       const int k = P >> 1, ph = k % K::NPH;
       if ((P & 1) != g) { it += K::nbox(ph); continue; }
-      const int img0 = (q / K::NSL) * K::IMGS, n0 = (q % K::NSL) * 64;
+      const int img0 = (q / K::NU) * K::IMGS, n0 = slice0(q);
       if (item_of(P - 1) >= 0) named_bar_sync(2 + g, 256);
       if (ph == 0) {
         for (int cb = 0; cb < K::CB && ok; ++cb) {
@@ -445,7 +476,7 @@
             if (cb > 0 || bb > 0) {
               wg_wait<1>();
               __syncwarp();
-              if (lane == 0) tc_mbar_arrive(&empty[(it - 1) % K::STAGES]);
+              if (lane == 0) release(it - 1);
             }
           }
         }
@@ -463,81 +494,110 @@
           if (cb > 0) {
             wg_wait<1>();
             __syncwarp();
-            if (lane == 0) tc_mbar_arrive(&empty[(it - 1) % K::STAGES]);
+            if (lane == 0) release(it - 1);
           }
         }
       }
       if (item_of(P + 1) >= 0) named_bar_arrive(3 - g, 256);
 
-      const uint16_t* rsrc = a.res + ((size_t)img0 * K::HW + pbase) * CI + n0 + 16 * wl + 8 * gh;
+      const uint16_t* rsrc = a.res + (size_t)img0 * K::HW * CI + n0 + 16 * wl + 8 * gh;
       uint4 rbuf[K::PF][2];
       if (S == 1 && a.res && ok) {
 #pragma unroll
         for (int p = 0; p < K::PF; ++p)
 #pragma unroll
           for (int e = 0; e < 2; ++e)
-            rbuf[p][e] = img0 + im_of(e) < a.N ? __ldg(reinterpret_cast<const uint4*>(rsrc + (size_t)(im_of(e) * K::HW + p * RSTEP + e * ESTEP) * CI))
-                                               : make_uint4(0u, 0u, 0u, 0u);
+            rbuf[p][e] = img0 + rimg(p, e) < a.N ? __ldg(reinterpret_cast<const uint4*>(rsrc + (size_t)rpix(p, e) * CI))
+                                                 : make_uint4(0u, 0u, 0u, 0u);
       }
       wg_wait<0>();
       __syncwarp();
-      if (ok && lane == 0) tc_mbar_arrive(&empty[(it - 1) % K::STAGES]);
-
-      float sm[K::IMGS], ss[K::IMGS];
-#pragma unroll
-      for (int im = 0; im < K::IMGS; ++im) { sm[im] = 0.f; ss[im] = 0.f; }
+      if (ok && lane == 0) release(it - 1);
+
+      float sm[K::TI], ss[K::TI];
+#pragma unroll
+      for (int t = 0; t < K::TI; ++t) { sm[t] = 0.f; ss[t] = 0.f; }
 #pragma unroll
       for (int j = 0; j < 32; ++j) {
         const float* d = &acc[4 * j];
-        sm[j % K::IMGS] += (d[0] + d[1]) + (d[2] + d[3]);
-        ss[j % K::IMGS] += (d[0] * d[0] + d[1] * d[1]) + (d[2] * d[2] + d[3] * d[3]);
-      }
-      float* rw = red + (((k & 1) * 2 + g) * 4) * K::IMGS * 2;
-#pragma unroll
-      for (int im = 0; im < K::IMGS; ++im) {
-        sm[im] = warp_sum(sm[im]); ss[im] = warp_sum(ss[im]);
-        if (lane == 0) *reinterpret_cast<float2*>(rw + (wl * K::IMGS + im) * 2) = make_float2(sm[im], ss[im]);
+        sm[j % K::TI] += (d[0] + d[1]) + (d[2] + d[3]);
+        ss[j % K::TI] += (d[0] * d[0] + d[1] * d[1]) + (d[2] * d[2] + d[3] * d[3]);
+      }
+      float* rw = red + ((K::RSL == 2 ? (k & 1) * 2 + g : g) * 4) * K::IMGS * 2;
+#pragma unroll
+      for (int t = 0; t < K::TI; ++t) {
+        if constexpr (WO >= 8) {
+          sm[t] = warp_sum(sm[t]); ss[t] = warp_sum(ss[t]);
+        } else {
+          sm[t] = warp_sum_skip2(sm[t]); ss[t] = warp_sum_skip2(ss[t]);
+        }
+        if (lane == 0 || (WO < 8 && lane == 2))
+          *reinterpret_cast<float2*>(rw + (wl * K::IMGS + img_of(t)) * 2) = make_float2(sm[t], ss[t]);
       }
       named_bar_sync(4 + g, 128);
+      float gs[K::TI], gss[K::TI];
+#pragma unroll
+      for (int t = 0; t < K::TI; ++t) {
+        gs[t] = 0.f; gss[t] = 0.f;
+#pragma unroll
+        for (int w = 0; w < K::GW; ++w) {
+          const float2 v = *reinterpret_cast<const float2*>(rw + ((grp * K::WPG + w) * K::IMGS + img_of(t)) * 2);
+          gs[t] += v.x; gss[t] += v.y;
+        }
+      }
+      if constexpr (K::XG) {
+        const int xq = 2 * g + (k & 1);
+        const float* xs = xch + xq * K::IMGS * 2;
+        if (ok) {
+          if (tid == 0) tc_mbar_expect_tx(&xbar[xq], (uint32_t)(K::IMGS * 2 * 4));
+          if (tid < 2 * K::IMGS) {
+            float v = 0.f;
+#pragma unroll
+            for (int w = 0; w < 4; ++w) v += rw[(w * K::IMGS + (tid >> 1)) * 2 + (tid & 1)];
+            uint32_t rdst, rbar;
+            asm volatile("mapa.shared::cluster.u32 %0, %1, %2;" : "=r"(rdst) : "r"(smem_u32(xs + tid)), "r"(rank ^ 1));
+            asm volatile("mapa.shared::cluster.u32 %0, %1, %2;" : "=r"(rbar) : "r"(smem_u32(&xbar[xq])), "r"(rank ^ 1));
+            asm volatile("st.async.shared::cluster.mbarrier::complete_tx::bytes.b32 [%0], %1, [%2];"
+                         ::"r"(rdst), "r"(__float_as_uint(v)), "r"(rbar) : "memory");
+          }
+        }
+        named_bar_sync(4 + g, 128);
+        if (ok) ok = tc_mbar_wait_cluster(&xbar[xq], (uint32_t)(k >> 1) & 1u, a.error);
+#pragma unroll
+        for (int t = 0; t < K::TI; ++t) { gs[t] += xs[img_of(t) * 2]; gss[t] += xs[img_of(t) * 2 + 1]; }
+      }
       if (!ok) continue;
-      float mean[K::IMGS], rstd[K::IMGS];
-#pragma unroll
-      for (int im = 0; im < K::IMGS; ++im) {
-        float s0 = 0.f, s1 = 0.f;
-#pragma unroll
-        for (int w = 0; w < K::WPG; ++w) {
-          const float2 v = *reinterpret_cast<const float2*>(rw + ((grp * K::WPG + w) * K::IMGS + im) * 2);
-          s0 += v.x; s1 += v.y;
-        }
-        mean[im] = s0 / count;
-        rstd[im] = rsqrtf(fmaxf(s1 / count - mean[im] * mean[im], 0.f) + a.eps);
+      float mean[K::TI], rstd[K::TI];
+#pragma unroll
+      for (int t = 0; t < K::TI; ++t) {
+        mean[t] = gs[t] / count;
+        rstd[t] = rsqrtf(fmaxf(gss[t] / count - mean[t] * mean[t], 0.f) + a.eps);
       }
 
       const float* gam = ph ? a.gamma_p : a.gamma;
       const float* bet = ph ? a.beta_p : a.beta;
       const bool relu = S == 2 ? ph == 0 : a.relu != 0;
       const bool rnorm = S == 1 && a.res_stats;
-      float ga[K::IMGS][2], gb[K::IMGS][2], ra[K::IMGS][2], rb[K::IMGS][2];
-#pragma unroll
-      for (int im = 0; im < K::IMGS; ++im) {
-        float rmean = 0.f, rrstd = 1.f;
-        if (rnorm && img0 + im < a.N) {
-          const float* rs = a.res_stats + ((size_t)(img0 + im) * 4 + n0 / K::CG) * 2;
-          rmean = rs[0] / count;
-          rrstd = rsqrtf(fmaxf(rs[1] / count - rmean * rmean, 0.f) + a.eps);
-        }
-#pragma unroll
-        for (int h = 0; h < 2; ++h) {
-          const int c = n0 + cl + 8 * h;
-          ga[im][h] = rstd[im] * gam[c];
-          gb[im][h] = bet[c] - mean[im] * ga[im][h];
-          ra[im][h] = rnorm ? rrstd * a.res_gamma[c] : 1.f;
-          rb[im][h] = rnorm ? a.res_beta[c] - rmean * ra[im][h] : 0.f;
-        }
+      float rmean[K::TI], rrstd[K::TI], gch[2], bch[2], rgch[2], rbch[2];
+#pragma unroll
+      for (int t = 0; t < K::TI; ++t) {
+        rmean[t] = 0.f; rrstd[t] = 1.f;
+        if (rnorm && img0 + img_of(t) < a.N) {
+          const float* rs = a.res_stats + ((size_t)(img0 + img_of(t)) * 4 + n0 / K::CG) * 2;
+          rmean[t] = rs[0] / count;
+          rrstd[t] = rsqrtf(fmaxf(rs[1] / count - rmean[t] * rmean[t], 0.f) + a.eps);
+        }
+      }
+#pragma unroll
+      for (int h = 0; h < 2; ++h) {
+        const int c = n0 + cl + 8 * h;
+        gch[h] = gam[c]; bch[h] = bet[c];
+        rgch[h] = rnorm ? a.res_gamma[c] : 1.f; rbch[h] = rnorm ? a.res_beta[c] : 0.f;
       }
 
       uint16_t* out = S == 2 && ph ? a.r : a.y;
-      const size_t obase = ((size_t)img0 * K::HW + pbase) * K::CO + n0 + 16 * wl + 8 * gh;
+      float* fbase = a.out_f32 + ((size_t)(img0 + img_of(0)) * K::HW + fpx) * CI + n0 + cl;
+      const size_t obase = (size_t)img0 * K::HW * K::CO + n0 + 16 * wl + 8 * gh;
 #pragma unroll
       for (int rd = 0; rd < 8; ++rd) {
         uint32_t rv[2][4];
@@ -550,8 +610,8 @@
           if (rd + K::PF < 8) {
 #pragma unroll
             for (int e = 0; e < 2; ++e)
-              if (img0 + im_of(e) < a.N)
-                rbuf[rd % K::PF][e] = __ldg(reinterpret_cast<const uint4*>(rsrc + (size_t)(im_of(e) * K::HW + (rd + K::PF) * RSTEP + e * ESTEP) * CI));
+              if (img0 + rimg(rd + K::PF, e) < a.N)
+                rbuf[rd % K::PF][e] = __ldg(reinterpret_cast<const uint4*>(rsrc + (size_t)rpix(rd + K::PF, e) * CI));
           }
         }
         uint32_t o[2][4];
@@ -559,19 +619,21 @@
         for (int x = 0; x < 2; ++x)
 #pragma unroll
           for (int jj = 0; jj < 2; ++jj) {
-            const int j = 4 * rd + 2 * x + jj, im = j % K::IMGS;
+            const int j = 4 * rd + 2 * x + jj, t = j % K::TI;
 #pragma unroll
             for (int h = 0; h < 2; ++h) {
               const float* d = &acc[4 * j + 2 * h];
-              float o0 = fmaf(d[0], ga[im][h], gb[im][h]), o1 = fmaf(d[1], ga[im][h], gb[im][h]);
+              const float ga = rstd[t] * gch[h], gb = bch[h] - mean[t] * ga;
+              float o0 = fmaf(d[0], ga, gb), o1 = fmaf(d[1], ga, gb);
               if (S == 1 && a.res) {
                 const float2 r = F::unpack(rv[x][2 * jj + h]);
-                o0 += fmaf(r.x, ra[im][h], rb[im][h]);
-                o1 += fmaf(r.y, ra[im][h], rb[im][h]);
+                const float ra = rrstd[t] * rgch[h], rb = rbch[h] - rmean[t] * ra;
+                o0 += fmaf(r.x, ra, rb);
+                o1 += fmaf(r.y, ra, rb);
               }
               if (relu) { o0 = fmaxf(o0, 0.f); o1 = fmaxf(o1, 0.f); }
-              if (S == 1 && a.out_f32 && img0 + im < a.N) {
-                float* of = a.out_f32 + ((size_t)(img0 + im) * K::HW + 8 * (j / K::IMGS) + 2 * (lane & 3)) * CI + n0 + cl + 8 * h;
+              if (S == 1 && a.out_f32 && img0 + img_of(t) < a.N) {
+                float* of = fbase + ((WO >= 8 ? t : 2 * t) * K::HW + (8 * j / (K::IMGS * WO)) * WO + 8 * j % WO) * CI + 8 * h;
                 of[0] = o0;
                 of[CI] = o1;
               }
@@ -585,14 +647,14 @@
           __syncwarp();
 #pragma unroll
           for (int e = 0; e < 2; ++e)
-            if (img0 + im_of(e) < a.N)
-              *reinterpret_cast<uint4*>(out + obase + (size_t)(im_of(e) * K::HW + rd * RSTEP + e * ESTEP) * K::CO) =
-                  *reinterpret_cast<const uint4*>(stg + grow + e * 512);
+            if (img0 + rimg(rd, e) < a.N)
+              *reinterpret_cast<uint4*>(out + obase + (size_t)rpix(rd, e) * K::CO) = *reinterpret_cast<const uint4*>(stg + grow + e * 512);
           __syncwarp();
         }
       }
     }
   }
+  if constexpr (K::CL > 1) cluster_sync_all();
 }
 
 template <class F, int S, int WO, int CI>
@@ -602,12 +664,24 @@
   static int slots = 0;
   if (!slots) {
     if (cudaFuncSetAttribute(kern, cudaFuncAttributeMaxDynamicSharedMemorySize, K::SMEM) != cudaSuccess) return check_launch("cudaFuncSetAttribute(conv3x3_pp)");
-    int dev = 0, sms = 0, per_sm = 0;
+    int dev = 0, sms = 0, n = 0;
     cudaGetDevice(&dev);
     cudaDeviceGetAttribute(&sms, cudaDevAttrMultiProcessorCount, dev);
-    if (cudaOccupancyMaxActiveBlocksPerMultiprocessor(&per_sm, kern, CONV_THREADS, K::SMEM) != cudaSuccess) return check_launch("cudaOccupancyMaxActiveBlocksPerMultiprocessor(conv3x3_pp)");
-    if (per_sm <= 0) { set_last_error("%s: conv3x3_pp_kernel (%d B shared memory) cannot be resident", name, K::SMEM); return SERL_ERR_CUDA; }
-    slots = per_sm * sms;
+    if (K::CL > 1) {
+      cudaLaunchConfig_t cfg = {};
+      cudaLaunchAttribute attr[1];
+      attr[0].id = cudaLaunchAttributeClusterDimension;
+      attr[0].val.clusterDim.x = K::CL; attr[0].val.clusterDim.y = 1; attr[0].val.clusterDim.z = 1;
+      cfg.gridDim = dim3(K::CL * sms); cfg.blockDim = dim3(CONV_THREADS); cfg.dynamicSmemBytes = K::SMEM;
+      cfg.attrs = attr; cfg.numAttrs = 1;
+      if (cudaOccupancyMaxActiveClusters(&n, kern, &cfg) != cudaSuccess) return check_launch("cudaOccupancyMaxActiveClusters(conv3x3_pp)");
+    } else {
+      int per_sm = 0;
+      if (cudaOccupancyMaxActiveBlocksPerMultiprocessor(&per_sm, kern, CONV_THREADS, K::SMEM) != cudaSuccess) return check_launch("cudaOccupancyMaxActiveBlocksPerMultiprocessor(conv3x3_pp)");
+      n = per_sm * sms;
+    }
+    if (n <= 0) { set_last_error("%s: conv3x3_pp_kernel (%d B shared memory) cannot be resident", name, K::SMEM); return SERL_ERR_CUDA; }
+    slots = n;
   }
   TcEncodeTiledFn enc = tc_get_encode();
   if (!enc) { set_last_error("%s: cuTensorMapEncodeTiled unavailable", name); return SERL_ERR_CUDA; }
@@ -634,9 +708,9 @@
     if (r != CUDA_SUCCESS) { set_last_error("%s: cuTensorMapEncodeTiled (weights) failed (%d)", name, (int)r); return SERL_ERR_CUDA; }
   }
   if (S == 1) pmap = wmap;
-  const int items = ceil_div(a.N, K::IMGS) * K::NSL;
+  const int items = ceil_div(a.N, K::IMGS) * K::NU;
   const int rounds = ceil_div(items, slots);
-  launch_k(kern, dim3(ceil_div(items, rounds)), dim3(CONV_THREADS), (size_t)K::SMEM, st, xmap, wmap, pmap, a);
+  launch_k_cluster(kern, dim3(K::CL * ceil_div(items, rounds)), dim3(CONV_THREADS), K::CL, (size_t)K::SMEM, st, xmap, wmap, pmap, a);
   return check_launch("conv3x3_pp_kernel");
 }
 
@@ -649,578 +723,14 @@
   return launch_conv3x3_pp<F, 2, WO, CI>("serl_conv3x3s2_res_h16", d->x, d->w, d->w_proj, d->fmt, a, st);
 }
 
-template <class F>
-static int launch_conv3x3_res8_pp(const serl_conv3x3_res_desc* d, cudaStream_t st) {
+template <class F, int W, int CI>
+static int launch_conv3x3_res_pp(const serl_conv3x3_res_desc* d, cudaStream_t st) {
   PPArgs a{};
   a.out_f32 = d->out_f32; a.y = d->out_f32 ? nullptr : static_cast<uint16_t*>(d->y);
   a.res = static_cast<const uint16_t*>(d->res); a.gamma = d->gamma; a.beta = d->beta;
   a.res_stats = d->res_stats; a.res_gamma = d->res_gamma; a.res_beta = d->res_beta;
   a.error = d->error; a.N = d->N; a.relu = d->relu; a.eps = d->eps;
-  return launch_conv3x3_pp<F, 1, 8, 256>("serl_conv3x3_res_h16", d->x, d->w, nullptr, d->fmt, a, st);
-}
-
-template <int WO, int CI>
-struct S2Cfg {
-  static constexpr int CO = 2 * CI;
-  static constexpr int BN = 128;
-  static constexpr int M = 128;
-  static constexpr int HW = WO * WO;
-  static constexpr int IMGS = M / HW;
-  static constexpr int NSL = CO / BN;
-  static constexpr int CB = CI / 64;
-  static constexpr int NB = 9;
-  static constexpr int NBOX = NB * CB;
-  static constexpr int BOX = IMGS * HW * 128;
-  static constexpr int TILE = BN * 128;
-  static constexpr int STAGE = BOX + 2 * TILE;
-  static constexpr int STAGES = 4;
-  static constexpr int CG = CO / 4;
-  static constexpr int CGS = 64;
-  static constexpr int GPS = 64 / CGS;
-  static constexpr int NGC = BN / CG;
-  static constexpr int OFF_STG = STAGES * STAGE;
-  static constexpr int OFF_PAR = OFF_STG + 8 * 1024;
-  static constexpr int OFF_RED = OFF_PAR + BN * 16;
-  static constexpr int OFF_ST = OFF_RED + 8 * 2 * GPS * 16;
-  static constexpr int OFF_BAR = OFF_ST + IMGS * NGC * 16;
-  static constexpr int SMEM = OFF_BAR + 8 * 2 * STAGES + 1024;
-  static_assert(WO == 4 && BN % CG == 0, "conv3x3s2_res_kernel: the WO 4 head, an item holds whole GroupNorm groups");
-  static_assert(M % HW == 0 && (BOX % 1024) == 0 && (STAGE % 1024) == 0 && SMEM <= 232448, "conv3x3s2_res_kernel: shared memory layout");
-  __device__ static constexpr int m_off(int wg, int) { return wg * 64; }
-  __device__ static constexpr int n_off(int h) { return h * 64; }
-};
-
-struct S2Args {
-  uint16_t* y; uint16_t* r; const float* gamma; const float* beta; const float* gamma_p; const float* beta_p;
-  int32_t* error; int N; float eps;
-};
-
-template <class F, int WO, int CI>
-__global__ void __launch_bounds__(CONV_THREADS, 1)
-conv3x3s2_res_kernel(const __grid_constant__ CUtensorMap xmap, const __grid_constant__ CUtensorMap wmap,
-                     const __grid_constant__ CUtensorMap pmap, const S2Args a) {
-  pdl_prologue();
-  using K = S2Cfg<WO, CI>;
-  extern __shared__ uint8_t smem_raw[];
-  uint8_t* smem = reinterpret_cast<uint8_t*>((reinterpret_cast<uintptr_t>(smem_raw) + 1023) & ~(uintptr_t)1023);
-  float* par = reinterpret_cast<float*>(smem + K::OFF_PAR);
-  float* red = reinterpret_cast<float*>(smem + K::OFF_RED);
-  float* gst = reinterpret_cast<float*>(smem + K::OFF_ST);
-  uint64_t* full = reinterpret_cast<uint64_t*>(smem + K::OFF_BAR);
-  uint64_t* empty = full + K::STAGES;
-
-  const int warp = threadIdx.x >> 5, lane = threadIdx.x & 31;
-  const int n_items = ceil_div(a.N, K::IMGS) * K::NSL;
-
-  if (threadIdx.x == 0) {
-    for (int s = 0; s < K::STAGES; ++s) { tc_mbar_init(&full[s], 1); tc_mbar_init(&empty[s], 8); }
-    asm volatile("fence.mbarrier_init.release.cluster;" ::: "memory");
-  }
-  __syncthreads();
-
-  if (warp >= 8) {
-    asm volatile("setmaxnreg.dec.sync.aligned.u32 40;" ::: "memory");
-    if (warp == 8 && lane == 0) {
-      asm volatile("prefetch.tensormap [%0];" ::"l"(&xmap) : "memory");
-      asm volatile("prefetch.tensormap [%0];" ::"l"(&wmap) : "memory");
-      asm volatile("prefetch.tensormap [%0];" ::"l"(&pmap) : "memory");
-      bool ok = true;
-      int it = 0;
-      for (int item = blockIdx.x; item < n_items && ok; item += gridDim.x) {
-        const int img = (item / K::NSL) * K::IMGS, n0 = (item % K::NSL) * K::BN;
-        for (int b = 0; b < K::NBOX; ++b, ++it) {
-          const int s = it % K::STAGES;
-          ok = tc_mbar_wait(&empty[s], ((uint32_t)(it / K::STAGES) & 1u) ^ 1u, a.error);
-          if (!ok) break;
-          const int cb = b / K::NB, row = (b % K::NB) / 3, sx = b % 3;
-          const bool proj = row == 0 && sx == 0;
-          uint8_t* st = smem + s * K::STAGE;
-          tc_mbar_expect_tx(&full[s], (uint32_t)(K::BOX + (1 + (int)proj) * K::TILE));
-          tc_tma_4d(st, &xmap, cb * 64, sx, row, img, &full[s]);
-          tc_tma_2d(st + K::BOX, &wmap, ((row * 3 + sx) * K::CB + cb) * 64, n0, &full[s]);
-          if (proj) tc_tma_2d(st + K::BOX + K::TILE, &pmap, cb * 64, n0, &full[s]);
-        }
-      }
-    }
-  } else {
-    asm volatile("setmaxnreg.inc.sync.aligned.u32 232;" ::: "memory");
-    const int tid = threadIdx.x, wg = tid >> 7, wl = warp & 3;
-    const uint32_t s_base = smem_u32(smem);
-    uint32_t a_off[2], b_off[2];
-#pragma unroll
-    for (int h = 0; h < 2; ++h) {
-      const int m = K::m_off(wg, h);
-      a_off[h] = (uint32_t)(m * 128);
-      b_off[h] = (uint32_t)(K::n_off(h) * 128);
-    }
-    const float count = (float)K::HW * (float)K::CG;
-    bool ok = true;
-    int it = 0;
-    float acc[2][32], pacc[2][32];
-    for (int item = blockIdx.x; item < n_items && ok; item += gridDim.x) {
-      const int img0 = (item / K::NSL) * K::IMGS, n0 = (item % K::NSL) * K::BN;
-      for (int cb = 0; cb < K::CB && ok; ++cb) {
-#pragma unroll
-        for (int bb = 0; bb < K::NB; ++bb, ++it) {
-          const int s = it % K::STAGES;
-          ok = tc_mbar_wait(&full[s], (uint32_t)(it / K::STAGES) & 1u, a.error);
-          if (!ok) break;
-          const uint32_t as = s_base + (uint32_t)(s * K::STAGE), ws = as + (uint32_t)K::BOX;
-          wg_fence();
-#pragma unroll
-          for (int k = 0; k < 4; ++k)
-#pragma unroll
-            for (int h = 0; h < 2; ++h)
-              wg_mma_h16<F::kBf16>(acc[h], wg_desc(as + a_off[h]) + 2 * k, wg_desc(ws + b_off[h]) + 2 * k, (uint32_t)(cb | bb | k));
-          if (bb == 0) {
-#pragma unroll
-            for (int k = 0; k < 4; ++k)
-#pragma unroll
-              for (int h = 0; h < 2; ++h)
-                wg_mma_h16<F::kBf16>(pacc[h], wg_desc(as + a_off[h]) + 2 * k, wg_desc(ws + (uint32_t)K::TILE + b_off[h]) + 2 * k,
-                                     (uint32_t)(cb | k));
-          }
-          wg_commit();
-          if (cb > 0 || bb > 0) {
-            wg_wait<1>();
-            __syncwarp();
-            if (lane == 0) tc_mbar_arrive(&empty[(it - 1) % K::STAGES]);
-          }
-        }
-      }
-      wg_wait<0>();
-      ok = mma_bar_and(ok);
-      if (!ok) break;
-      __syncwarp();
-      if (lane == 0) tc_mbar_arrive(&empty[(it - 1) % K::STAGES]);
-
-#pragma unroll
-      for (int h = 0; h < 2; ++h)
-#pragma unroll
-        for (int g = 0; g < K::GPS; ++g) {
-          float v[4] = {0.f, 0.f, 0.f, 0.f};
-#pragma unroll
-          for (int j = g * K::CGS / 8; j < (g + 1) * K::CGS / 8; ++j) {
-            const float* d = &acc[h][4 * j];
-            const float* p = &pacc[h][4 * j];
-            v[0] += (d[0] + d[1]) + (d[2] + d[3]);
-            v[1] += (d[0] * d[0] + d[1] * d[1]) + (d[2] * d[2] + d[3] * d[3]);
-            v[2] += (p[0] + p[1]) + (p[2] + p[3]);
-            v[3] += (p[0] * p[0] + p[1] * p[1]) + (p[2] * p[2] + p[3] * p[3]);
-          }
-#pragma unroll
-          for (int q = 0; q < 4; ++q) {
-            v[q] = warp_sum(v[q]);
-            if (lane == 0) red[((warp * 2 + h) * K::GPS + g) * 4 + q] = v[q];
-          }
-        }
-      asm volatile("bar.sync 1, 256;" ::: "memory");
-      if (tid < K::BN)
-        *reinterpret_cast<float4*>(par + tid * 4) = make_float4(a.gamma[n0 + tid], a.beta[n0 + tid], a.gamma_p[n0 + tid], a.beta_p[n0 + tid]);
-      if (tid < K::IMGS * K::NGC) {
-        const int im = tid / K::NGC, gc = tid % K::NGC;
-        float S[4] = {0.f, 0.f, 0.f, 0.f};
-        for (int w = 0; w < 8; ++w)
-          for (int h = 0; h < 2; ++h)
-            for (int g = 0; g < K::GPS; ++g) {
-              if ((K::m_off(w >> 2, h) + 16 * (w & 3)) / K::HW != im || (K::n_off(h) + g * K::CGS) / K::CG != gc) continue;
-              for (int q = 0; q < 4; ++q) S[q] += red[((w * 2 + h) * K::GPS + g) * 4 + q];
-            }
-        const float mean = S[0] / count, pmean = S[2] / count;
-        const float var = fmaxf(S[1] / count - mean * mean, 0.f), pvar = fmaxf(S[3] / count - pmean * pmean, 0.f);
-        *reinterpret_cast<float4*>(gst + tid * 4) = make_float4(mean, rsqrtf(var + a.eps), pmean, rsqrtf(pvar + a.eps));
-      }
-      asm volatile("bar.sync 1, 256;" ::: "memory");
-
-      uint8_t* stg = smem + K::OFF_STG + warp * 1024;
-#pragma unroll
-      for (int h = 0; h < 2; ++h)
-#pragma unroll
-        for (int hf = 0; hf < 2; ++hf) {
-          const int m8 = K::m_off(wg, h) + wl * 16 + hf * 8;
-          const int im = m8 / K::HW;
-          if (img0 + im >= a.N) continue;
-          const int rr = lane >> 2;
-          const size_t pix0 = (size_t)img0 * K::HW + m8;
-#pragma unroll 1
-          for (int o = 0; o < 2; ++o) {
-#pragma unroll
-            for (int j = 0; j < 8; ++j) {
-              const int c = K::n_off(h) + 8 * j + 2 * (lane & 3);
-              const float4 sv = *reinterpret_cast<const float4*>(gst + (im * K::NGC + c / K::CG) * 4);
-              const float4 p0 = *reinterpret_cast<const float4*>(par + c * 4), p1 = *reinterpret_cast<const float4*>(par + c * 4 + 4);
-              float o0, o1;
-              if (o == 0) {
-                const float g0 = sv.y * p0.x, g1 = sv.y * p1.x;
-                o0 = fmaxf(fmaf(acc[h][4 * j + 2 * hf], g0, p0.y - sv.x * g0), 0.f);
-                o1 = fmaxf(fmaf(acc[h][4 * j + 2 * hf + 1], g1, p1.y - sv.x * g1), 0.f);
-              } else {
-                const float g0 = sv.w * p0.z, g1 = sv.w * p1.z;
-                o0 = fmaf(pacc[h][4 * j + 2 * hf], g0, p0.w - sv.z * g0);
-                o1 = fmaf(pacc[h][4 * j + 2 * hf + 1], g1, p1.w - sv.z * g1);
-              }
-              *reinterpret_cast<uint32_t*>(stg + rr * 128 + ((j ^ rr) << 4) + (lane & 3) * 4) = F::pack(o0, o1);
-            }
-            __syncwarp();
-            uint16_t* out = o == 0 ? a.y : a.r;
-#pragma unroll
-            for (int e = lane; e < 64; e += 32) {
-              const int q = e >> 3, ch = e & 7;
-              const uint4 v = *reinterpret_cast<const uint4*>(stg + q * 128 + ((ch ^ q) << 4));
-              *reinterpret_cast<uint4*>(out + (pix0 + q) * K::CO + n0 + K::n_off(h) + ch * 8) = v;
-            }
-            __syncwarp();
-          }
-        }
-    }
-  }
-}
-
-template <class F, int WO, int CI>
-static int launch_conv3x3s2_res(const serl_conv3x3s2_res_desc* d, cudaStream_t st) {
-  using K = S2Cfg<WO, CI>;
-  auto kern = conv3x3s2_res_kernel<F, WO, CI>;
-  static int slots = 0;
-  if (!slots) {
-    if (cudaFuncSetAttribute(kern, cudaFuncAttributeMaxDynamicSharedMemorySize, K::SMEM) != cudaSuccess) return check_launch("cudaFuncSetAttribute(conv3x3s2_res)");
-    int dev = 0, sms = 0, per_sm = 0;
-    cudaGetDevice(&dev);
-    cudaDeviceGetAttribute(&sms, cudaDevAttrMultiProcessorCount, dev);
-    if (cudaOccupancyMaxActiveBlocksPerMultiprocessor(&per_sm, kern, CONV_THREADS, K::SMEM) != cudaSuccess) return check_launch("cudaOccupancyMaxActiveBlocksPerMultiprocessor(conv3x3s2_res)");
-    if (per_sm <= 0) { set_last_error("serl_conv3x3s2_res_h16: conv3x3s2_res_kernel (%d B shared memory) cannot be resident", K::SMEM); return SERL_ERR_CUDA; }
-    slots = per_sm * sms;
-  }
-  TcEncodeTiledFn enc = tc_get_encode();
-  if (!enc) { set_last_error("serl_conv3x3s2_res_h16: cuTensorMapEncodeTiled unavailable"); return SERL_ERR_CUDA; }
-  const CUtensorMapDataType dt = d->fmt == SERL_FMT_FP16 ? CU_TENSOR_MAP_DATA_TYPE_FLOAT16 : CU_TENSOR_MAP_DATA_TYPE_BFLOAT16;
-  CUtensorMap xmap, wmap, pmap;
-  {
-    const cuuint64_t gdim[4] = {(cuuint64_t)CI, (cuuint64_t)(2 * WO), (cuuint64_t)(2 * WO), (cuuint64_t)d->N};
-    const cuuint64_t gstr[3] = {(cuuint64_t)CI * 2, (cuuint64_t)2 * WO * CI * 2, (cuuint64_t)4 * WO * WO * CI * 2};
-    const cuuint32_t box[4] = {64u, (cuuint32_t)(2 * WO), (cuuint32_t)(2 * WO), (cuuint32_t)K::IMGS};
-    const cuuint32_t estr[4] = {1u, 2u, 2u, 1u};
-    CUresult r = enc(&xmap, dt, 4, const_cast<void*>(d->x), gdim, gstr, box, estr, CU_TENSOR_MAP_INTERLEAVE_NONE, CU_TENSOR_MAP_SWIZZLE_128B,
-                     CU_TENSOR_MAP_L2_PROMOTION_L2_256B, CU_TENSOR_MAP_FLOAT_OOB_FILL_NONE);
-    if (r != CUDA_SUCCESS) { set_last_error("serl_conv3x3s2_res_h16: cuTensorMapEncodeTiled (input) failed (%d)", (int)r); return SERL_ERR_CUDA; }
-  }
-  for (int pj = 0; pj < 2; ++pj) {
-    const cuuint64_t kdim = (cuuint64_t)(pj ? 1 : 9) * CI;
-    const cuuint64_t gdim[2] = {kdim, (cuuint64_t)K::CO};
-    const cuuint64_t gstr[1] = {kdim * 2};
-    const cuuint32_t box[2] = {64u, (cuuint32_t)K::BN};
-    const cuuint32_t estr[2] = {1u, 1u};
-    CUresult r = enc(pj ? &pmap : &wmap, dt, 2, const_cast<void*>(pj ? d->w_proj : d->w), gdim, gstr, box, estr, CU_TENSOR_MAP_INTERLEAVE_NONE,
-                     CU_TENSOR_MAP_SWIZZLE_128B, CU_TENSOR_MAP_L2_PROMOTION_L2_256B, CU_TENSOR_MAP_FLOAT_OOB_FILL_NONE);
-    if (r != CUDA_SUCCESS) { set_last_error("serl_conv3x3s2_res_h16: cuTensorMapEncodeTiled (weights) failed (%d)", (int)r); return SERL_ERR_CUDA; }
-  }
-  S2Args a{};
-  a.y = static_cast<uint16_t*>(d->y); a.r = static_cast<uint16_t*>(d->r);
-  a.gamma = d->gamma; a.beta = d->beta; a.gamma_p = d->gamma_proj; a.beta_p = d->beta_proj;
-  a.error = d->error; a.N = d->N; a.eps = d->eps;
-  const int items = ceil_div(d->N, K::IMGS) * K::NSL;
-  const int rounds = ceil_div(items, slots);
-  launch_k(kern, dim3(ceil_div(items, rounds)), dim3(CONV_THREADS), (size_t)K::SMEM, st, xmap, wmap, pmap, a);
-  return check_launch("conv3x3s2_res_kernel");
-}
-
-template <int W, int CI>
-struct DeepCfg {
-  static constexpr int BN = 128;
-  static constexpr int HW = W * W;
-  static constexpr int IMGS = 256 / HW;
-  static constexpr int NSL = CI / BN;
-  static constexpr int CB = CI / 64;
-  static constexpr int NB = 9;
-  static constexpr int NBOX = NB * CB;
-  static constexpr int BOX = IMGS * HW * 128;
-  static constexpr int TILE = BN * 128;
-  static constexpr int STAGE = BOX + TILE;
-  static constexpr int STAGES = 4;
-  static constexpr int RES = 128 * 128 * 2;
-  static constexpr int RPS = STAGE / RES;
-  static constexpr int NRES = 2 / RPS;
-  static constexpr int CG = CI / 4;
-  static constexpr int NGC = BN / CG;
-  static constexpr int OFF_STG = STAGES * STAGE;
-  static constexpr int OFF_PAR = OFF_STG + 8 * 2048;
-  static constexpr int OFF_RED = OFF_PAR + BN * 16;
-  static constexpr int OFF_ST = OFF_RED + 8 * 2 * 2 * 8;
-  static constexpr int OFF_BAR = OFF_ST + IMGS * NGC * 16;
-  static constexpr int SMEM = OFF_BAR + 8 * 2 * STAGES + 1024;
-  static_assert(CG >= 64 && BN % CG == 0, "conv3x3_deep_kernel: an n64 sub-tile lies in one group, an item holds whole groups");
-  static_assert(RPS >= 1 && NRES < STAGES, "conv3x3_deep_kernel: the residual fits the ring");
-  static_assert(HW >= 16 && (BOX % 1024) == 0 && (STAGE % 1024) == 0 && SMEM <= 232448, "conv3x3_deep_kernel: shared memory layout");
-  __device__ static constexpr int m_off(int wg, int h) { return wg * 128 + h * 64; }
-};
-
-struct DeepArgs {
-  uint16_t* y; float* out_f32; const uint16_t* res; const float* gamma; const float* beta;
-  const float* res_stats; const float* res_gamma; const float* res_beta;
-  int32_t* error; int N, relu; float eps;
-};
-
-template <class F, int W, int CI>
-__global__ void __launch_bounds__(CONV_THREADS, 1)
-conv3x3_deep_kernel(const __grid_constant__ CUtensorMap xmap, const __grid_constant__ CUtensorMap wmap,
-                    const __grid_constant__ CUtensorMap rmap, const DeepArgs a) {
-  pdl_prologue();
-  using K = DeepCfg<W, CI>;
-  extern __shared__ uint8_t smem_raw[];
-  uint8_t* smem = reinterpret_cast<uint8_t*>((reinterpret_cast<uintptr_t>(smem_raw) + 1023) & ~(uintptr_t)1023);
-  float* par = reinterpret_cast<float*>(smem + K::OFF_PAR);
-  float* red = reinterpret_cast<float*>(smem + K::OFF_RED);
-  float* gst = reinterpret_cast<float*>(smem + K::OFF_ST);
-  uint64_t* full = reinterpret_cast<uint64_t*>(smem + K::OFF_BAR);
-  uint64_t* empty = full + K::STAGES;
-
-  const int warp = threadIdx.x >> 5, lane = threadIdx.x & 31;
-  const int n_items = ceil_div(a.N, K::IMGS) * K::NSL;
-
-  if (threadIdx.x == 0) {
-    for (int s = 0; s < K::STAGES; ++s) { tc_mbar_init(&full[s], 1); tc_mbar_init(&empty[s], 8); }
-    asm volatile("fence.mbarrier_init.release.cluster;" ::: "memory");
-  }
-  __syncthreads();
-
-  if (warp >= 8) {
-    asm volatile("setmaxnreg.dec.sync.aligned.u32 40;" ::: "memory");
-    if (warp == 8 && lane == 0) {
-      asm volatile("prefetch.tensormap [%0];" ::"l"(&xmap) : "memory");
-      asm volatile("prefetch.tensormap [%0];" ::"l"(&wmap) : "memory");
-      if (a.res) asm volatile("prefetch.tensormap [%0];" ::"l"(&rmap) : "memory");
-      bool ok = true;
-      int it = 0;
-      for (int item = blockIdx.x; item < n_items && ok; item += gridDim.x) {
-        const int img = (item / K::NSL) * K::IMGS, n0 = (item % K::NSL) * K::BN;
-        for (int b = 0; b < K::NBOX + (a.res ? K::NRES : 0); ++b, ++it) {
-          const int s = it % K::STAGES;
-          ok = tc_mbar_wait(&empty[s], ((uint32_t)(it / K::STAGES) & 1u) ^ 1u, a.error);
-          if (!ok) break;
-          uint8_t* st = smem + s * K::STAGE;
-          if (b >= K::NBOX) {
-            tc_mbar_expect_tx(&full[s], (uint32_t)(K::RPS * K::RES));
-            for (int q = 0; q < K::RPS; ++q)
-              for (int c = 0; c < 2; ++c)
-                tc_tma_2d(st + q * K::RES + c * (K::RES / 2), &rmap, n0 + c * 64, img * K::HW + ((b - K::NBOX) * K::RPS + q) * 128, &full[s]);
-            continue;
-          }
-          const int cb = b / K::NB, row = (b % K::NB) / 3, sx = b % 3;
-          tc_mbar_expect_tx(&full[s], (uint32_t)K::STAGE);
-          tc_tma_4d(st, &xmap, cb * 64, sx - 1, row - 1, img, &full[s]);
-          tc_tma_2d(st + K::BOX, &wmap, ((row * 3 + sx) * K::CB + cb) * 64, n0, &full[s]);
-        }
-      }
-    }
-  } else {
-    asm volatile("setmaxnreg.inc.sync.aligned.u32 232;" ::: "memory");
-    const int tid = threadIdx.x, wg = tid >> 7, wl = warp & 3;
-    const uint32_t s_base = smem_u32(smem);
-    uint32_t a_off[2];
-#pragma unroll
-    for (int h = 0; h < 2; ++h) a_off[h] = (uint32_t)(K::m_off(wg, h) * 128);
-    const float count = (float)K::HW * (float)K::CG;
-    bool ok = true;
-    int it = 0;
-    float acc[2][2][32];
-    for (int item = blockIdx.x; item < n_items && ok; item += gridDim.x) {
-      const int img0 = (item / K::NSL) * K::IMGS, n0 = (item % K::NSL) * K::BN;
-      for (int cb = 0; cb < K::CB && ok; ++cb) {
-#pragma unroll
-        for (int bb = 0; bb < K::NB; ++bb, ++it) {
-          const int s = it % K::STAGES;
-          ok = tc_mbar_wait(&full[s], (uint32_t)(it / K::STAGES) & 1u, a.error);
-          if (!ok) break;
-          const uint32_t as = s_base + (uint32_t)(s * K::STAGE), ws = as + (uint32_t)K::BOX;
-          wg_fence();
-#pragma unroll
-          for (int k = 0; k < 4; ++k)
-#pragma unroll
-            for (int h = 0; h < 2; ++h)
-#pragma unroll
-              for (int c = 0; c < 2; ++c)
-                wg_mma_h16<F::kBf16>(acc[h][c], wg_desc(as + a_off[h]) + 2 * k, wg_desc(ws + (uint32_t)(c * 64 * 128)) + 2 * k,
-                                     (uint32_t)(cb | bb | k));
-          wg_commit();
-          if (cb > 0 || bb > 0) {
-            wg_wait<1>();
-            __syncwarp();
-            if (lane == 0) tc_mbar_arrive(&empty[(it - 1) % K::STAGES]);
-          }
-        }
-      }
-      wg_wait<0>();
-      ok = mma_bar_and(ok);
-      if (!ok) break;
-      __syncwarp();
-      if (lane == 0) tc_mbar_arrive(&empty[(it - 1) % K::STAGES]);
-
-#pragma unroll
-      for (int h = 0; h < 2; ++h)
-#pragma unroll
-        for (int c = 0; c < 2; ++c) {
-          float v0 = 0.f, v1 = 0.f;
-#pragma unroll
-          for (int j = 0; j < 8; ++j) {
-            const float* d = &acc[h][c][4 * j];
-            v0 += (d[0] + d[1]) + (d[2] + d[3]);
-            v1 += (d[0] * d[0] + d[1] * d[1]) + (d[2] * d[2] + d[3] * d[3]);
-          }
-          v0 = warp_sum(v0); v1 = warp_sum(v1);
-          if (lane == 0) *reinterpret_cast<float2*>(red + ((warp * 2 + h) * 2 + c) * 2) = make_float2(v0, v1);
-        }
-      asm volatile("bar.sync 1, 256;" ::: "memory");
-      if (tid < K::BN) {
-        const int ch = n0 + tid;
-        *reinterpret_cast<float4*>(par + tid * 4) = a.res_stats ? make_float4(a.gamma[ch], a.beta[ch], a.res_gamma[ch], a.res_beta[ch])
-                                                                : make_float4(a.gamma[ch], a.beta[ch], 1.f, 0.f);
-      }
-      if (tid < K::IMGS * K::NGC) {
-        const int im = tid / K::NGC, gc = tid % K::NGC;
-        float S = 0.f, SS = 0.f;
-        for (int w = 0; w < 8; ++w)
-          for (int h = 0; h < 2; ++h)
-            for (int c = 0; c < 2; ++c) {
-              if ((K::m_off(w >> 2, h) + 16 * (w & 3)) / K::HW != im || c * 64 / K::CG != gc) continue;
-              S += red[((w * 2 + h) * 2 + c) * 2];
-              SS += red[((w * 2 + h) * 2 + c) * 2 + 1];
-            }
-        const float mean = S / count;
-        const float var = fmaxf(SS / count - mean * mean, 0.f);
-        float rmean = 0.f, rrstd = 1.f;
-        if (a.res_stats && img0 + im < a.N) {
-          const float* rs = a.res_stats + ((size_t)(img0 + im) * 4 + (n0 / K::CG + gc)) * 2;
-          rmean = rs[0] / count;
-          rrstd = rsqrtf(fmaxf(rs[1] / count - rmean * rmean, 0.f) + a.eps);
-        }
-        *reinterpret_cast<float4*>(gst + tid * 4) = make_float4(mean, rsqrtf(var + a.eps), rmean, rrstd);
-      }
-      const int rpos = it + wg / K::RPS;
-      const uint8_t* rsm = smem + (rpos % K::STAGES) * K::STAGE + (wg % K::RPS) * K::RES;
-      if (a.res) ok = tc_mbar_wait(&full[rpos % K::STAGES], (uint32_t)(rpos / K::STAGES) & 1u, a.error);
-      ok = mma_bar_and(ok);
-      if (!ok) break;
-
-      uint8_t* stg = smem + K::OFF_STG + warp * 2048;
-      const int rr = lane >> 2;
-#pragma unroll
-      for (int h = 0; h < 2; ++h)
-#pragma unroll
-        for (int hf = 0; hf < 2; ++hf) {
-          const int m8 = K::m_off(wg, h) + wl * 16 + hf * 8;
-          const int im = m8 / K::HW;
-          if (img0 + im >= a.N) continue;
-          const size_t pix0 = (size_t)img0 * K::HW + m8;
-#pragma unroll
-          for (int c = 0; c < 2; ++c) {
-            const float4 sv = *reinterpret_cast<const float4*>(gst + (im * K::NGC + c * 64 / K::CG) * 4);
-#pragma unroll
-            for (int j = 0; j < 8; ++j) {
-              const int cl = c * 64 + 8 * j + 2 * (lane & 3);
-              const float4 p0 = *reinterpret_cast<const float4*>(par + cl * 4), p1 = *reinterpret_cast<const float4*>(par + cl * 4 + 4);
-              const float g0 = sv.y * p0.x, g1 = sv.y * p1.x;
-              float o0 = fmaf(acc[h][c][4 * j + 2 * hf], g0, p0.y - sv.x * g0);
-              float o1 = fmaf(acc[h][c][4 * j + 2 * hf + 1], g1, p1.y - sv.x * g1);
-              if (a.res) {
-                const float2 rv = F::unpack(*reinterpret_cast<const uint32_t*>(
-                    rsm + c * (K::RES / 2) + (m8 - wg * 128 + rr) * 128 + ((j ^ rr) << 4) + (lane & 3) * 4));
-                if (a.res_stats) {
-                  const float r0 = sv.w * p0.z, r1 = sv.w * p1.z;
-                  o0 += fmaf(rv.x, r0, p0.w - sv.z * r0);
-                  o1 += fmaf(rv.y, r1, p1.w - sv.z * r1);
-                } else {
-                  o0 += rv.x; o1 += rv.y;
-                }
-              }
-              if (a.relu) { o0 = fmaxf(o0, 0.f); o1 = fmaxf(o1, 0.f); }
-              if (a.out_f32)
-                *reinterpret_cast<float2*>(stg + rr * 256 + ((j ^ rr) << 5) + (lane & 3) * 8) = make_float2(o0, o1);
-              else
-                *reinterpret_cast<uint32_t*>(stg + rr * 128 + ((j ^ rr) << 4) + (lane & 3) * 4) = F::pack(o0, o1);
-            }
-            __syncwarp();
-            if (a.out_f32) {
-#pragma unroll
-              for (int e = lane; e < 128; e += 32) {
-                const int q = e >> 4, ch = e & 15;
-                const uint4 v = *reinterpret_cast<const uint4*>(stg + q * 256 + (((ch >> 1) ^ q) << 5) + (ch & 1) * 16);
-                *reinterpret_cast<uint4*>(a.out_f32 + (pix0 + q) * CI + n0 + c * 64 + ch * 4) = v;
-              }
-            } else {
-#pragma unroll
-              for (int e = lane; e < 64; e += 32) {
-                const int q = e >> 3, ch = e & 7;
-                const uint4 v = *reinterpret_cast<const uint4*>(stg + q * 128 + ((ch ^ q) << 4));
-                *reinterpret_cast<uint4*>(a.y + (pix0 + q) * CI + n0 + c * 64 + ch * 8) = v;
-              }
-            }
-            __syncwarp();
-          }
-        }
-      if (a.res) {
-        __syncwarp();
-        if (lane == 0)
-          for (int p = 0; p < K::NRES; ++p) tc_mbar_arrive(&empty[(it + p) % K::STAGES]);
-        it += K::NRES;
-      }
-    }
-  }
-}
-
-template <class F, int W, int CI>
-static int launch_conv3x3_deep(const serl_conv3x3_res_desc* d, cudaStream_t st) {
-  using K = DeepCfg<W, CI>;
-  auto kern = conv3x3_deep_kernel<F, W, CI>;
-  static int slots = 0;
-  if (!slots) {
-    if (cudaFuncSetAttribute(kern, cudaFuncAttributeMaxDynamicSharedMemorySize, K::SMEM) != cudaSuccess) return check_launch("cudaFuncSetAttribute(conv3x3_deep)");
-    int dev = 0, sms = 0, per_sm = 0;
-    cudaGetDevice(&dev);
-    cudaDeviceGetAttribute(&sms, cudaDevAttrMultiProcessorCount, dev);
-    if (cudaOccupancyMaxActiveBlocksPerMultiprocessor(&per_sm, kern, CONV_THREADS, K::SMEM) != cudaSuccess) return check_launch("cudaOccupancyMaxActiveBlocksPerMultiprocessor(conv3x3_deep)");
-    if (per_sm <= 0) { set_last_error("serl_conv3x3_res_h16: conv3x3_deep_kernel (%d B shared memory) cannot be resident", K::SMEM); return SERL_ERR_CUDA; }
-    slots = per_sm * sms;
-  }
-  TcEncodeTiledFn enc = tc_get_encode();
-  if (!enc) { set_last_error("serl_conv3x3_res_h16: cuTensorMapEncodeTiled unavailable"); return SERL_ERR_CUDA; }
-  const CUtensorMapDataType dt = d->fmt == SERL_FMT_FP16 ? CU_TENSOR_MAP_DATA_TYPE_FLOAT16 : CU_TENSOR_MAP_DATA_TYPE_BFLOAT16;
-  CUtensorMap xmap, wmap, rmap;
-  {
-    const cuuint64_t gdim[4] = {(cuuint64_t)CI, (cuuint64_t)W, (cuuint64_t)W, (cuuint64_t)d->N};
-    const cuuint64_t gstr[3] = {(cuuint64_t)CI * 2, (cuuint64_t)W * CI * 2, (cuuint64_t)W * W * CI * 2};
-    const cuuint32_t box[4] = {64u, (cuuint32_t)W, (cuuint32_t)W, (cuuint32_t)K::IMGS};
-    const cuuint32_t estr[4] = {1u, 1u, 1u, 1u};
-    CUresult r = enc(&xmap, dt, 4, const_cast<void*>(d->x), gdim, gstr, box, estr, CU_TENSOR_MAP_INTERLEAVE_NONE, CU_TENSOR_MAP_SWIZZLE_128B,
-                     CU_TENSOR_MAP_L2_PROMOTION_L2_256B, CU_TENSOR_MAP_FLOAT_OOB_FILL_NONE);
-    if (r != CUDA_SUCCESS) { set_last_error("serl_conv3x3_res_h16: cuTensorMapEncodeTiled (input) failed (%d)", (int)r); return SERL_ERR_CUDA; }
-  }
-  {
-    const cuuint64_t gdim[2] = {(cuuint64_t)9 * CI, (cuuint64_t)CI};
-    const cuuint64_t gstr[1] = {(cuuint64_t)9 * CI * 2};
-    const cuuint32_t box[2] = {64u, (cuuint32_t)K::BN};
-    const cuuint32_t estr[2] = {1u, 1u};
-    CUresult r = enc(&wmap, dt, 2, const_cast<void*>(d->w), gdim, gstr, box, estr, CU_TENSOR_MAP_INTERLEAVE_NONE, CU_TENSOR_MAP_SWIZZLE_128B,
-                     CU_TENSOR_MAP_L2_PROMOTION_L2_256B, CU_TENSOR_MAP_FLOAT_OOB_FILL_NONE);
-    if (r != CUDA_SUCCESS) { set_last_error("serl_conv3x3_res_h16: cuTensorMapEncodeTiled (weights) failed (%d)", (int)r); return SERL_ERR_CUDA; }
-  }
-  rmap = wmap;
-  if (d->res) {
-    const cuuint64_t gdim[2] = {(cuuint64_t)CI, (cuuint64_t)d->N * W * W};
-    const cuuint64_t gstr[1] = {(cuuint64_t)CI * 2};
-    const cuuint32_t box[2] = {64u, 128u};
-    const cuuint32_t estr[2] = {1u, 1u};
-    CUresult r = enc(&rmap, dt, 2, const_cast<void*>(d->res), gdim, gstr, box, estr, CU_TENSOR_MAP_INTERLEAVE_NONE, CU_TENSOR_MAP_SWIZZLE_128B,
-                     CU_TENSOR_MAP_L2_PROMOTION_L2_256B, CU_TENSOR_MAP_FLOAT_OOB_FILL_NONE);
-    if (r != CUDA_SUCCESS) { set_last_error("serl_conv3x3_res_h16: cuTensorMapEncodeTiled (residual) failed (%d)", (int)r); return SERL_ERR_CUDA; }
-  }
-  DeepArgs a{};
-  a.out_f32 = d->out_f32; a.y = d->out_f32 ? nullptr : static_cast<uint16_t*>(d->y);
-  a.res = static_cast<const uint16_t*>(d->res); a.gamma = d->gamma; a.beta = d->beta;
-  a.res_stats = d->res_stats; a.res_gamma = d->res_gamma; a.res_beta = d->res_beta;
-  a.error = d->error; a.N = d->N; a.relu = d->relu; a.eps = d->eps;
-  const int items = ceil_div(d->N, K::IMGS) * K::NSL;
-  const int rounds = ceil_div(items, slots);
-  launch_k(kern, dim3(ceil_div(items, rounds)), dim3(CONV_THREADS), (size_t)K::SMEM, st, xmap, wmap, rmap, a);
-  return check_launch("conv3x3_deep_kernel");
+  return launch_conv3x3_pp<F, 1, W, CI>("serl_conv3x3_res_h16", d->x, d->w, nullptr, d->fmt, a, st);
 }
 
 }
@@ -1239,7 +749,7 @@
   const cudaStream_t st = static_cast<cudaStream_t>(stream);
   if (d->Wo == 16) return h ? launch_conv3x3s2_pp<Fp16, 16, 64>(d, st) : launch_conv3x3s2_pp<Bf16, 16, 64>(d, st);
   if (d->Wo == 8) return h ? launch_conv3x3s2_pp<Fp16, 8, 128>(d, st) : launch_conv3x3s2_pp<Bf16, 8, 128>(d, st);
-  return h ? launch_conv3x3s2_res<Fp16, 4, 256>(d, st) : launch_conv3x3s2_res<Bf16, 4, 256>(d, st);
+  return h ? launch_conv3x3s2_pp<Fp16, 4, 256>(d, st) : launch_conv3x3s2_pp<Bf16, 4, 256>(d, st);
 }
 
 extern "C" int serl_conv3x3_res_h16(const serl_conv3x3_res_desc* d, void* stream) {
@@ -1266,9 +776,9 @@
                                    : launch_conv3x3_res<Bf16, 16, 128>(d, static_cast<cudaStream_t>(stream));
   }
   if (d->W == 8) {
-    return d->fmt == SERL_FMT_FP16 ? launch_conv3x3_res8_pp<Fp16>(d, static_cast<cudaStream_t>(stream))
-                                   : launch_conv3x3_res8_pp<Bf16>(d, static_cast<cudaStream_t>(stream));
-  }
-  return d->fmt == SERL_FMT_FP16 ? launch_conv3x3_deep<Fp16, 4, 512>(d, static_cast<cudaStream_t>(stream))
-                                 : launch_conv3x3_deep<Bf16, 4, 512>(d, static_cast<cudaStream_t>(stream));
-}
+    return d->fmt == SERL_FMT_FP16 ? launch_conv3x3_res_pp<Fp16, 8, 256>(d, static_cast<cudaStream_t>(stream))
+                                   : launch_conv3x3_res_pp<Bf16, 8, 256>(d, static_cast<cudaStream_t>(stream));
+  }
+  return d->fmt == SERL_FMT_FP16 ? launch_conv3x3_res_pp<Fp16, 4, 512>(d, static_cast<cudaStream_t>(stream))
+                               : launch_conv3x3_res_pp<Bf16, 4, 512>(d, static_cast<cudaStream_t>(stream));
+}
diff --git a/serl_b200/csrc/conv_common.cuh b/serl_b200/csrc/conv_common.cuh
--- a/serl_b200/csrc/conv_common.cuh
+++ b/serl_b200/csrc/conv_common.cuh
@@ -81,6 +81,16 @@
   asm volatile("cp.async.bulk.tensor.4d.shared::cluster.global.tile.mbarrier::complete_tx::bytes [%0], [%1, {%3, %4, %5, %6}], [%2];"
                ::"r"(smem_u32(smem_dst)), "l"(map), "r"(smem_u32(bar)), "r"(c0), "r"(c1), "r"(c2), "r"(c3) : "memory");
 }
+__device__ inline void tc_tma_4d_mc(void* smem_dst, const CUtensorMap* map, int c0, int c1, int c2, int c3, uint64_t* bar, uint16_t cta_mask) {
+  asm volatile("cp.async.bulk.tensor.4d.shared::cluster.global.tile.mbarrier::complete_tx::bytes.multicast::cluster"
+               " [%0], [%1, {%3, %4, %5, %6}], [%2], %7;"
+               ::"r"(smem_u32(smem_dst)), "l"(map), "r"(smem_u32(bar)), "r"(c0), "r"(c1), "r"(c2), "r"(c3), "h"(cta_mask) : "memory");
+}
+__device__ inline void tc_mbar_arrive_remote(uint64_t* bar, uint32_t rank) {
+  uint32_t addr;
+  asm volatile("mapa.shared::cluster.u32 %0, %1, %2;" : "=r"(addr) : "r"(smem_u32(bar)), "r"(rank));
+  asm volatile("mbarrier.arrive.shared::cluster.b64 _, [%0];" ::"r"(addr) : "memory");
+}
 
 constexpr int CONV_THREADS = 384;
 
```

After: 546.0 (median of 6 runs). About the same (+0.8%).
